# manuelbb-upb/Morbit.jl

Hardware: AMD Instinct MI355X
Metric: RBF build+solve+eval cycles/sec (higher is better)
Workload: dtype f64

## Files before the change

include/mrbf.h:

```cpp
#ifndef MRBF_H
#define MRBF_H

#include <stdint.h>

#ifdef __cplusplus
extern "C" {
#endif

typedef struct mrbf_ctx mrbf_ctx;
typedef struct mrbf_model mrbf_model;

enum {
    MRBF_CUBIC = 0,
    MRBF_INV_MULTIQUADRIC = 1,
    MRBF_MULTIQUADRIC = 2,
    MRBF_THIN_PLATE_SPLINE = 3,
    MRBF_GAUSSIAN = 4
};

enum {
    MRBF_OK = 0,
    MRBF_ENOTPD = 1,
    MRBF_ESINGULAR = 2,
    MRBF_EHIP = 3,
// ... 151 lines not shown
    const double *X;
    double *weights_out;
    double *poly_out;
    double *vals_out;
    double *jac_out;
} mrbf_problem;

typedef struct {
    int32_t status;
    int32_t device;
    mrbf_fit_info fit;
    float ms_eval;
    double checksum_w;
    double checksum_vals;
} mrbf_result;

int32_t mrbf_batch_run(int32_t n_dev, const int32_t *device_ids, int64_t n_problems, const mrbf_problem *problems,
                       mrbf_result *results);

typedef struct {
    int64_t n;
    int32_t d, k, kernel_id, poly_deg;
    double a, b;
    const double *centres, *values;
    double *weights_out, *poly_out;
    mrbf_model *model;
    int32_t status;
    int32_t reserved;
    mrbf_fit_info info;
} mrbf_fit_job;
int32_t mrbf_fit_batch(mrbf_ctx *ctx, int64_t n_starts, mrbf_fit_job *jobs, float *ms_total);

typedef struct {
    const mrbf_model *model;
    int64_t m;
    const double *X;
    double *vals_out;
    double *jac_out;
    int32_t status;
    int32_t reserved;
} mrbf_eval_job;
int32_t mrbf_eval_batch(mrbf_ctx *ctx, int64_t n_jobs, mrbf_eval_job *jobs, float *ms_total);
int32_t mrbf_eval_batch_limited(mrbf_ctx *ctx, int64_t n_jobs, mrbf_eval_job *jobs, float *ms_total, int64_t arena_limit_bytes);

typedef struct {
    const mrbf_model *model;
    int64_t m;
    const double *X;
    const int32_t *rows;
    double *hess_out;
    int32_t n_rows;
    int32_t status;
    int32_t nsplit;
    int32_t reserved;
} mrbf_hess_job;
typedef struct {
    float ms_total;
    int32_t chunks;
    int32_t groups;
    int32_t single_inside;
} mrbf_hess_batch_info;
int32_t mrbf_eval_hessian_batch(mrbf_ctx *ctx, int64_t n_jobs, mrbf_hess_job *jobs, mrbf_hess_batch_info *info);
int32_t mrbf_eval_hessian_batch_limited(mrbf_ctx *ctx, int64_t n_jobs, mrbf_hess_job *jobs, mrbf_hess_batch_info *info,
                                        int64_t arena_limit_bytes);

typedef struct mrbf_db mrbf_db;
int32_t mrbf_db_create(mrbf_ctx *ctx, int32_t d, int32_t k, int64_t capacity_hint, mrbf_db **db);
int32_t mrbf_db_append(mrbf_ctx *ctx, mrbf_db *db, int64_t m, const double *sites, const double *values, int64_t *first_index);
int32_t mrbf_db_set_values(mrbf_ctx *ctx, mrbf_db *db, int64_t m, const int64_t *indices, const double *values);
int32_t mrbf_db_read(mrbf_ctx *ctx, const mrbf_db *db, int64_t first, int64_t m, double *sites_out, double *values_out);
int32_t mrbf_db_dims(const mrbf_db *db, int64_t *n_sites, int32_t *d, int32_t *k);
int32_t mrbf_db_free(mrbf_ctx *ctx, mrbf_db *db);

typedef struct {
    mrbf_db *db;
    const double *lb, *ub, *x0;
    int64_t n_exclude;
    const int64_t *exclude;
    int32_t zero_first_pick;
    int32_t rc;
    int64_t *indices_out;
    double *sites_out, *shifted_out;
    double *first_row;
    int64_t mc;
    int64_t first_pick;
    const double *cand_sites_dev;
    const double *shifted_dev;
} mrbf_db_box_job;
int32_t mrbf_db_box_batch(mrbf_ctx *ctx, int64_t n_starts, int32_t d, int32_t p_is_inf, mrbf_db_box_job *jobs, float *ms_total);

typedef struct {
    mrbf_db *db;
    int64_t n_idx;
    const int64_t *indices;
    double *sites_out, *values_out;
    const double *sites_dev;
    const double *values_dev;
    int32_t rc;
    int32_t reserved;
} mrbf_db_gather_job;
int32_t mrbf_db_gather_batch(mrbf_ctx *ctx, int64_t n_starts, int32_t d, mrbf_db_gather_job *jobs, float *ms_total);

typedef struct {
    mrbf_db *db;
    int64_t m;
    const double *sites;
    const double *values;
    int64_t first_index;
    int32_t rc;
    int32_t reserved;
} mrbf_db_append_job;
int32_t mrbf_db_append_batch(mrbf_ctx *ctx, int64_t n_starts, mrbf_db_append_job *jobs, float *ms_total);
typedef struct {
    mrbf_db *db;
    int64_t m;
    const int64_t *indices;
    const double *values;
    int32_t rc;
    int32_t reserved;
} mrbf_db_set_values_job;
int32_t mrbf_db_set_values_batch(mrbf_ctx *ctx, int64_t n_starts, mrbf_db_set_values_job *jobs, float *ms_total);

enum { MRBF_R3_UPDATE = 0, MRBF_R3_IMPROVE = 1 };
enum { MRBF_R3_DONE = 0, MRBF_R3_REBUILT = 1 };
typedef struct {
    mrbf_db *db;
    const double *x, *lb, *ub;
    double pivot_val;
    const double *dirs;
    int32_t n_dirs, reversed;
    int32_t n_missing, max_new;
    int32_t ensure_fully_linear, force_rebuild, mode;
    int32_t rc;
    double *new_sites_out;
    int64_t first_index;
    int32_t n_new, fully_linear, status, n_dirs_used;
} mrbf_round3_job;
int32_t mrbf_db_round3_batch(mrbf_ctx *ctx, int64_t n_starts, int32_t d, mrbf_round3_job *jobs, float *ms_total);

int32_t mrbf_debug_env(const char *name);
int32_t mrbf_debug_mfma_layout(mrbf_ctx *ctx, double *out16x16_a_times_b, const double *A16x4, const double *B4x16);
int32_t mrbf_debug_potrf(mrbf_ctx *ctx, int64_t n, double *A_colmajor_inout, int32_t impl, int32_t *info, float *ms);
int32_t mrbf_debug_diag(mrbf_ctx *ctx, const double *A128, int32_t reps, float *ms_per_call, double *shader_cycles,
                        double *realtime_us);
int32_t mrbf_debug_mfma_peak(mrbf_ctx *ctx, int32_t blocks_per_cu, int32_t threads, int32_t iters, float *ms, double *tflops);
int32_t mrbf_debug_mfma_asm(mrbf_ctx *ctx, int32_t variant, int32_t blocks_per_cu, int32_t iters, float *ms, double *tflops,
                            double *cycles_per_mfma);
int32_t mrbf_debug_dgemm(mrbf_ctx *ctx, int32_t m, int32_t n, int32_t k, float *ms, double *tflops);
int32_t mrbf_debug_mega_tables(int32_t nt, int32_t mt, int32_t slack, int32_t slack_chain, int32_t first, int32_t win, int32_t srows,
                               int32_t half_cols, int64_t *out6);
int32_t mrbf_debug_mega_tables2(int32_t nt, int32_t mt, int32_t slack, int32_t slack_chain, int32_t first, int32_t win, int32_t srows,
                                int32_t half_cols, const int32_t *opt5, int64_t *out6);
int32_t mrbf_debug_mega_plan(int32_t nt, int32_t mt, int32_t xreal, int64_t *out39);

enum { MRBF_PS_OK = 0, MRBF_PS_CRITICAL = 1, MRBF_PS_FAILURE = 2 };
typedef struct {
    int32_t max_ideal_evals;
    int32_t max_ps_evals;
    int32_t max_polish_evals;
    int32_t reserved;
    uint64_t seed;
    double t0;
    double xtol_rel;
} mrbf_ps_options;
typedef struct {
    int32_t status;
    int32_t generations;
    int32_t evals_ideal, evals_ps, evals_polish;
    float ms_total;
    double tau;
} mrbf_ps_info;
int32_t mrbf_ps_step(mrbf_ctx *ctx, const mrbf_model *model, const double *x_n, const double *lb_eff, const double *ub_eff,
                     const double *fx_n, const double *r_or_null, const mrbf_ps_options *opts, double *x_trial, double *mx_trial,
                     double *r_out, mrbf_ps_info *info);

enum { MRBF_ROLE_NONE = -1, MRBF_ROLE_EQ = -2, MRBF_ROLE_INEQ = -3 };
typedef struct {
    int32_t n_models, n_objectives;
    const mrbf_model *const *models;
    const int32_t *roles;
    int32_t n_lin_eq, n_lin_ineq;
    const double *A_eq, *b_eq, *A_ineq, *b_ineq;
    double eq_tol;
} mrbf_ps_problem;
int32_t mrbf_ps_step_problem(mrbf_ctx *ctx, const mrbf_ps_problem *problem, const double *x_n, const double *lb_eff,
                             const double *ub_eff, const double *fx_n, const double *r_or_null, const mrbf_ps_options *opts,
                             double *x_trial, double *mx_trial, double *r_out, mrbf_ps_info *info);
int32_t mrbf_debug_ps_rank(mrbf_ctx *ctx, int32_t lam, const double *f, const double *phi, uint64_t seed, int32_t gen, int32_t impl,
                           int32_t *order_out, int32_t *gave_up);

enum { MRBF_SD_OK = 0, MRBF_SD_NO_OBJECTIVE = 1, MRBF_SD_INFEASIBLE = 2, MRBF_SD_GAVE_UP = 3 };
int32_t mrbf_sd_direction(mrbf_ctx *ctx, int64_t n_lp, int32_t d, int32_t k, int32_t m_eq, int32_t m_ineq, const double *G,
                          const double *x, const double *lb, const double *ub, const double *A_eq, const double *b_eq,
                          const double *A_ineq, const double *b_ineq, int32_t normalize, double *d_out, double *omega_out,
                          double *dual_out, int32_t *status_out, int32_t *iters_out);
typedef struct {
    int32_t status;
    int32_t iterations;
    int32_t bound_flips;
    float ms_total;
    double omega;
} mrbf_sd_info;
int32_t mrbf_sd_criticality(mrbf_ctx *ctx, const mrbf_ps_problem *problem, const double *x, const double *x_n, const double *lb,
                            const double *ub, int32_t normalize, double *d_out, double *dual_out, mrbf_sd_info *info);

enum { MRBF_NS_OK = 0, MRBF_NS_INFEASIBLE = 1, MRBF_NS_GAVE_UP = 2 };
int32_t mrbf_normal_direction(mrbf_ctx *ctx, int64_t n_lp, int32_t d, int32_t m_eq, int32_t m_ineq, const double *x, const double *lb,
                              const double *ub, const double *A_eq, const double *b_eq, const double *A_ineq, const double *b_ineq,
                              double *n_out, double *alpha_out, double *dual_out, int32_t *status_out, int32_t *iters_out);
typedef struct {
    int32_t status;
    int32_t iterations;
    int32_t bound_flips;
    float ms_total;
    double alpha;
    double delta;
} mrbf_normal_info;
int32_t mrbf_normal_step(mrbf_ctx *ctx, const mrbf_ps_problem *problem, int32_t d, const double *x, const double *lb, const double *ub,
                         double delta, double kappa_delta, double delta_max, int32_t variable_radius, double *n_out, double *dual_out,
                         mrbf_normal_info *info);

typedef struct {
    int32_t strict;
    int32_t max_loops;
    double const_rhs;
    double shrink;
    double min_stepsize;
} mrbf_sd_step_options;
typedef struct {
    int32_t branch;
    int32_t loops;
    float ms_total;
    double sigma;
    double omega;
    double step_norm;
} mrbf_sd_step_info;
int32_t mrbf_sd_step(mrbf_ctx *ctx, const mrbf_ps_problem *problem, const double *x, const double *x_n, double delta, const double *lb,
                     const double *ub, double omega, const double *d, const mrbf_sd_step_options *opts, double *x_plus, double *mx_plus,
                     mrbf_sd_step_info *info);

typedef struct {
    int32_t sd_status;
    int32_t iterations, bound_flips;
    int32_t branch, loops;
    int32_t reserved;
    double omega;
    double omega_step;
    double sigma, step_norm;
} mrbf_sd_batch_record;
int32_t mrbf_sd_iterate_batch(mrbf_ctx *ctx, int64_t n_starts, const mrbf_ps_problem *shape, const mrbf_model *const *models,
                              const double *x, const double *x_n, const double *delta, const double *lb, const double *ub,
                              int32_t normalize, const mrbf_sd_step_options *opts, double *d_out, double *x_plus, double *mx_plus,
                              mrbf_sd_batch_record *records, float *ms_total);

typedef struct {
    int32_t status;
    int32_t iterations, bound_flips;
    int32_t reserved;
    double alpha;
    double delta;
} mrbf_normal_batch_record;
int32_t mrbf_normal_step_batch(mrbf_ctx *ctx, int64_t n_starts, const mrbf_ps_problem *shape, const mrbf_model *const *models, int32_t d,
                               const double *x, const double *lb, const double *ub, const double *delta, double kappa_delta,
                               double delta_max, int32_t variable_radius, double *n_out, double *x_n_out, double *dual_out,
                               mrbf_normal_batch_record *records, float *ms_total);

int32_t mrbf_ps_step_batch(mrbf_ctx *ctx, int64_t n_starts, const mrbf_ps_problem *shape, const mrbf_model *const *models,
                           const double *x_n, const double *lb_eff, const double *ub_eff, const double *fx_n, const double *r_or_null,
                           const mrbf_ps_options *opts, const uint64_t *seeds_or_null, double *x_trial, double *mx_trial, double *r_out,
                           mrbf_ps_info *infos, float *ms_total);

enum { MRBF_DISPATCH_REFERENCE = 0, MRBF_DISPATCH_DEVICE = 1 };
enum { MRBF_FIT_FULL = 0, MRBF_FIT_FROM_ROUND4 = 1 };
enum { MRBF_ENTRY_ROUND4 = 1, MRBF_ENTRY_FIT_FROM_ROUND4 = 2, MRBF_ENTRY_PS_STEP = 3, MRBF_ENTRY_BACKTRACK = 4, MRBF_ENTRY_AFFINE = 5,
       MRBF_ENTRY_SD = 6, MRBF_ENTRY_NORMAL = 7, MRBF_ENTRY_SD_STEP = 8, MRBF_ENTRY_SD_BATCH = 9, MRBF_ENTRY_AFFINE_BATCH = 10,
       MRBF_ENTRY_FIT_BATCH = 11, MRBF_ENTRY_NORMAL_BATCH = 12, MRBF_ENTRY_ROUND4_BATCH = 13, MRBF_ENTRY_PS_BATCH = 14,
       MRBF_ENTRY_DB_BOX = 15, MRBF_ENTRY_DB_GATHER = 16, MRBF_ENTRY_DB_ROUND3 = 17, MRBF_ENTRY_DB_APPEND_BATCH = 18,
       MRBF_ENTRY_DB_SET_VALUES_BATCH = 19, MRBF_ENTRY_EVAL_BATCH = 20, MRBF_ENTRY_HESSIAN_BATCH = 21 };
int32_t mrbf_dispatch_ps(int32_t d, int32_t k, int32_t n_models, int32_t n_nl_constraints, int32_t n_lin_constraints, int32_t n_foreign);
int32_t mrbf_dispatch_ps_batch(int64_t n_starts, int32_t d, int32_t k, int32_t n_models, int32_t n_nl_constraints,
                               int32_t n_lin_constraints, int32_t n_foreign);
int32_t mrbf_dispatch_sd(int32_t d, int32_t k, int32_t n_models, int32_t n_nl_constraints, int32_t n_lin_constraints, int32_t n_foreign);
int32_t mrbf_dispatch_normal(int32_t d, int32_t n_models, int32_t n_nl_constraints, int32_t n_lin_constraints, int32_t n_foreign);
int32_t mrbf_dispatch_sd_step(int32_t d, int32_t k, int32_t n_models, int32_t n_nl_constraints, int32_t n_lin_constraints, int32_t n_foreign,
                              int32_t max_loops);
int32_t mrbf_dispatch_sd_batch(int64_t n_starts, int32_t d, int32_t k, int32_t n_models, int32_t n_nl_constraints,
                               int32_t n_lin_constraints, int32_t n_foreign, int32_t max_loops);
int32_t mrbf_dispatch_normal_batch(int64_t n_starts, int32_t d, int32_t n_models, int32_t n_nl_constraints, int32_t n_lin_constraints,
                                   int32_t n_foreign);
int32_t mrbf_dispatch_backtrack(int32_t n_objective_models, int32_t n_foreign, int32_t outputs_in_order);
int32_t mrbf_dispatch_affine(int64_t n_candidates, int32_t d);
int32_t mrbf_dispatch_affine_batch(int64_t n_starts, int32_t d, int32_t p_is_inf);
int32_t mrbf_dispatch_round4(int64_t n0, int32_t d, int32_t poly_deg, int64_t n_candidates);
int32_t mrbf_dispatch_fit_batch(int64_t n_starts);
int64_t mrbf_dispatch_fit_batch_max_n(int64_t n_starts, int32_t d);
int32_t mrbf_dispatch_fit_batch_lu(int64_t n_lu_starts, int64_t n_max, int32_t d);
int32_t mrbf_dispatch_round4_batch(int64_t n_starts, int32_t d);
int32_t mrbf_dispatch_db_batch(int64_t n_starts, int32_t d);
int32_t mrbf_dispatch_eval_batch(int64_t n_jobs);
int64_t mrbf_dispatch_eval_batch_min_jobs(void);
int32_t mrbf_dispatch_hessian_batch(int64_t n_jobs);
int64_t mrbf_dispatch_hessian_batch_min_jobs(void);
int32_t mrbf_dispatch_fit(int64_t n_training, int64_t state_n0, int32_t state_q, int32_t state_n_accepted, int32_t same_sites);
int32_t mrbf_dispatch_after(int32_t entry, int32_t rc);

int32_t mrbf_stochastic_rank(int32_t lam, const double *f, const double *phi, const double *u, double pf, int32_t *idx_out);
// ... 6 lines not shown
```

morbit.jl_amd/_lib.py:

```python
import ctypes
import os

import numpy as np

_HERE = os.path.dirname(os.path.abspath(__file__))
LIB_PATH = os.environ.get("MRBF_LIB") or os.path.join(_HERE, "libmrbf.so")

c_dp = ctypes.POINTER(ctypes.c_double)
c_fp = ctypes.POINTER(ctypes.c_float)
c_ip = ctypes.POINTER(ctypes.c_int32)
c_vp = ctypes.c_void_p

MRBF_OK, MRBF_ENOTPD, MRBF_ESINGULAR, MRBF_EHIP, MRBF_EBLAS, MRBF_ENOMEM, MRBF_ENODEVICE, MRBF_ENCCL = range(8)
PATH_CHOL, PATH_PROJ_CHOL, PATH_LU, PATH_MINNORM, PATH_ROUND4 = 1, 2, 3, 4, 5
OPT_GRAM_MODE, OPT_RESIDUAL, OPT_FORCE_PATH, OPT_CHOL_IMPL, OPT_EVAL_IMPL, OPT_TIMING, OPT_DIAG_IMPL, OPT_CHOL_WINDOW = 1, 2, 3, 4, 5, 6, 7, 8
OPT_SPIN_MS, OPT_DEBUG_FAULT, OPT_LAST_DEVICE_MS, OPT_SLOW_LAUNCHES = 9, 10, 11, 12
OPT_ARENA_BYTES, OPT_LIVE_HANDLES = 13, 14
OPT_SMALL_FIT_MAX_N = 15
SMALL_FIT_DEFAULT_MAX_N = 512
OPT_SMALL_LU = 16
SMALL_LU_MAX_N, SMALL_LU_MAX_D, SMALL_LU_MAX_K = 512, 128, 16
FB_CHOL_HOST_DRIVEN, FB_BACKSOLVE_BLOCKED, FB_LU = 1, 2, 4


# ... 126 lines not shown

    def asdict(self):
        return {f: getattr(self, f) for f, _ in self._fields_}


class AffineJob(ctypes.Structure):
    _fields_ = [("mc", ctypes.c_int64), ("j0", ctypes.c_int32), ("max_picks", ctypes.c_int32), ("pivot_val", ctypes.c_double),
                ("shifted", ctypes.c_void_p), ("Q0", ctypes.c_void_p), ("picked_out", ctypes.c_void_p), ("Z_out", ctypes.c_void_p),
                ("n_picked", ctypes.c_int32), ("reserved", ctypes.c_int32)]


class Round4Job(ctypes.Structure):
    _fields_ = [("n0", ctypes.c_int64), ("mc", ctypes.c_int64), ("start_sites", ctypes.c_void_p), ("cand_sites", ctypes.c_void_p),
                ("kernel_id", ctypes.c_int32), ("poly_deg", ctypes.c_int32), ("a", ctypes.c_double), ("b", ctypes.c_double),
                ("max_points", ctypes.c_int32), ("theta_pivot_cholesky", ctypes.c_double), ("accepted_out", ctypes.c_void_p),
                ("n_accepted", ctypes.c_int32), ("rc", ctypes.c_int32)]


class FitJob(ctypes.Structure):
    _fields_ = [("n", ctypes.c_int64), ("d", ctypes.c_int32), ("k", ctypes.c_int32), ("kernel_id", ctypes.c_int32),
                ("poly_deg", ctypes.c_int32), ("a", ctypes.c_double), ("b", ctypes.c_double), ("centres", ctypes.c_void_p),
                ("values", ctypes.c_void_p), ("weights_out", ctypes.c_void_p), ("poly_out", ctypes.c_void_p), ("model", ctypes.c_void_p),
                ("status", ctypes.c_int32), ("reserved", ctypes.c_int32), ("info", FitInfo)]


class EvalJob(ctypes.Structure):
    _fields_ = [("model", ctypes.c_void_p), ("m", ctypes.c_int64), ("X", ctypes.c_void_p), ("vals_out", ctypes.c_void_p),
                ("jac_out", ctypes.c_void_p), ("status", ctypes.c_int32), ("reserved", ctypes.c_int32)]


class DbBoxJob(ctypes.Structure):
    _fields_ = [("db", ctypes.c_void_p), ("lb", ctypes.c_void_p), ("ub", ctypes.c_void_p), ("x0", ctypes.c_void_p),
                ("n_exclude", ctypes.c_int64), ("exclude", ctypes.c_void_p), ("zero_first_pick", ctypes.c_int32), ("rc", ctypes.c_int32),
                ("indices_out", ctypes.c_void_p), ("sites_out", ctypes.c_void_p), ("shifted_out", ctypes.c_void_p),
                ("first_row", ctypes.c_void_p), ("mc", ctypes.c_int64), ("first_pick", ctypes.c_int64),
                ("cand_sites_dev", ctypes.c_void_p), ("shifted_dev", ctypes.c_void_p)]


class DbGatherJob(ctypes.Structure):
    _fields_ = [("db", ctypes.c_void_p), ("n_idx", ctypes.c_int64), ("indices", ctypes.c_void_p), ("sites_out", ctypes.c_void_p),
                ("values_out", ctypes.c_void_p), ("sites_dev", ctypes.c_void_p), ("values_dev", ctypes.c_void_p),
                ("rc", ctypes.c_int32), ("reserved", ctypes.c_int32)]


class DbAppendJob(ctypes.Structure):
    _fields_ = [("db", ctypes.c_void_p), ("m", ctypes.c_int64), ("sites", ctypes.c_void_p), ("values", ctypes.c_void_p),
                ("first_index", ctypes.c_int64), ("rc", ctypes.c_int32), ("reserved", ctypes.c_int32)]


class DbSetValuesJob(ctypes.Structure):
    _fields_ = [("db", ctypes.c_void_p), ("m", ctypes.c_int64), ("indices", ctypes.c_void_p), ("values", ctypes.c_void_p),
                ("rc", ctypes.c_int32), ("reserved", ctypes.c_int32)]


class Round3Job(ctypes.Structure):
    _fields_ = [("db", ctypes.c_void_p), ("x", ctypes.c_void_p), ("lb", ctypes.c_void_p), ("ub", ctypes.c_void_p),
                ("pivot_val", ctypes.c_double), ("dirs", ctypes.c_void_p), ("n_dirs", ctypes.c_int32), ("reversed", ctypes.c_int32),
                ("n_missing", ctypes.c_int32), ("max_new", ctypes.c_int32), ("ensure_fully_linear", ctypes.c_int32),
                ("force_rebuild", ctypes.c_int32), ("mode", ctypes.c_int32), ("rc", ctypes.c_int32), ("new_sites_out", ctypes.c_void_p),
                ("first_index", ctypes.c_int64), ("n_new", ctypes.c_int32), ("fully_linear", ctypes.c_int32), ("status", ctypes.c_int32),
                ("n_dirs_used", ctypes.c_int32)]


class Problem(ctypes.Structure):
    _fields_ = [("n", ctypes.c_int64), ("m", ctypes.c_int64), ("d", ctypes.c_int32), ("k", ctypes.c_int32),
                ("kernel_id", ctypes.c_int32), ("poly_deg", ctypes.c_int32), ("a", ctypes.c_double), ("b", ctypes.c_double),
                ("centres", c_dp), ("values", c_dp), ("X", c_dp), ("weights_out", c_dp), ("poly_out", c_dp),
                ("vals_out", c_dp), ("jac_out", c_dp)]


class Result(ctypes.Structure):
    _fields_ = [("status", ctypes.c_int32), ("device", ctypes.c_int32), ("fit", FitInfo), ("ms_eval", ctypes.c_float),
                ("checksum_w", ctypes.c_double), ("checksum_vals", ctypes.c_double)]


SIGNATURES = {
    "mrbf_init": (ctypes.c_int32, [ctypes.c_int32, ctypes.POINTER(c_vp)]),
    "mrbf_shutdown": (ctypes.c_int32, [c_vp]),
    "mrbf_last_error": (ctypes.c_char_p, [c_vp]),
    "mrbf_version": (ctypes.c_char_p, []),
    "mrbf_set_option": (ctypes.c_int32, [c_vp, ctypes.c_int32, ctypes.c_double]),
    "mrbf_get_option": (ctypes.c_int32, [c_vp, ctypes.c_int32, c_dp]),
    "mrbf_set_stream": (ctypes.c_int32, [c_vp, c_vp]),
    "mrbf_sync": (ctypes.c_int32, [c_vp]),
    "mrbf_gram": (ctypes.c_int32, [c_vp, ctypes.c_int64, ctypes.c_int32, c_vp, ctypes.c_int32, ctypes.c_double,
                                   ctypes.c_double, ctypes.c_int32, c_vp, c_vp, c_fp]),
    "mrbf_cross_gram": (ctypes.c_int32, [c_vp, ctypes.c_int64, ctypes.c_int64, ctypes.c_int32, c_vp, c_vp, ctypes.c_int32, ctypes.c_double,
                                         ctypes.c_double, c_vp]),
    "mrbf_fit": (ctypes.c_int32, [c_vp, ctypes.c_int64, ctypes.c_int32, ctypes.c_int32, c_vp, c_vp, ctypes.c_int32,
                                  ctypes.c_double, ctypes.c_double, ctypes.c_int32, ctypes.POINTER(c_vp), c_vp, c_vp,
                                  ctypes.POINTER(FitInfo)]),
    "mrbf_model_from_coeffs": (ctypes.c_int32, [c_vp, ctypes.c_int64, ctypes.c_int32, ctypes.c_int32, c_vp, c_vp, c_vp,
                                                ctypes.c_int32, ctypes.c_double, ctypes.c_double, ctypes.c_int32,
                                                ctypes.POINTER(c_vp)]),
    "mrbf_eval": (ctypes.c_int32, [c_vp, c_vp, ctypes.c_int64, c_vp, c_vp, c_vp, ctypes.POINTER(EvalInfo)]),
    "mrbf_eval_hessian": (ctypes.c_int32, [c_vp, c_vp, ctypes.c_int64, c_vp, ctypes.c_int32, c_vp, c_vp, ctypes.POINTER(HessInfo)]),
    "mrbf_eval_hessian_limited": (ctypes.c_int32, [c_vp, c_vp, ctypes.c_int64, c_vp, ctypes.c_int32, c_vp, c_vp, ctypes.POINTER(HessInfo),
                                                   ctypes.c_int64]),
    "mrbf_backtrack": (ctypes.c_int32, [c_vp, c_vp, c_vp, c_vp, ctypes.c_double, ctypes.c_double, ctypes.c_int32,
                                        ctypes.c_double, ctypes.c_double, ctypes.c_double, ctypes.c_int32, c_vp, c_vp,
                                        c_vp, c_ip]),
    "mrbf_affine_scores": (ctypes.c_int32, [c_vp, ctypes.c_int64, ctypes.c_int32, ctypes.c_int32, c_vp, c_vp, ctypes.c_int32, c_vp,
                                            ctypes.POINTER(ctypes.c_int64), c_dp]),
    "mrbf_affine_select": (ctypes.c_int32, [c_vp, ctypes.c_int64, ctypes.c_int32, c_vp, ctypes.c_int32, c_vp, ctypes.c_int32, ctypes.c_double,
                                            ctypes.c_int32, ctypes.POINTER(ctypes.c_int64), c_ip, c_vp]),
    "mrbf_affine_select_batch": (ctypes.c_int32, [c_vp, ctypes.c_int64, ctypes.c_int32, ctypes.c_int32, ctypes.POINTER(AffineJob), c_fp]),
    "mrbf_round4": (ctypes.c_int32, [c_vp, ctypes.c_int64, ctypes.c_int32, c_vp, ctypes.c_int64, c_vp, ctypes.c_int32, ctypes.c_double,
                                     ctypes.c_double, ctypes.c_int32, ctypes.c_int32, ctypes.c_double, c_vp, c_ip, ctypes.POINTER(c_vp)]),
    "mrbf_fit_from_round4": (ctypes.c_int32, [c_vp, c_vp, ctypes.c_int32, c_vp, ctypes.POINTER(c_vp), c_vp, c_vp, ctypes.POINTER(FitInfo)]),
    "mrbf_round4_sites": (ctypes.c_int32, [c_vp, ctypes.POINTER(ctypes.c_int64), ctypes.POINTER(ctypes.c_int64), c_ip]),
    "mrbf_free_round4": (ctypes.c_int32, [c_vp, c_vp]),
    "mrbf_round4_batch": (ctypes.c_int32, [c_vp, ctypes.c_int64, ctypes.c_int32, ctypes.POINTER(Round4Job), c_fp]),
    "mrbf_dispatch_round4_batch": (ctypes.c_int32, [ctypes.c_int64, ctypes.c_int32]),
    "mrbf_model_dims": (ctypes.c_int32, [c_vp, ctypes.POINTER(ctypes.c_int64), c_ip, c_ip, c_ip]),
    "mrbf_free_model": (ctypes.c_int32, [c_vp, c_vp]),
    "mrbf_batch_run": (ctypes.c_int32, [ctypes.c_int32, c_ip, ctypes.c_int64, ctypes.POINTER(Problem),
                                        ctypes.POINTER(Result)]),
    "mrbf_fit_batch": (ctypes.c_int32, [c_vp, ctypes.c_int64, ctypes.POINTER(FitJob), c_fp]),
    "mrbf_dispatch_fit_batch": (ctypes.c_int32, [ctypes.c_int64]),
    "mrbf_dispatch_fit_batch_max_n": (ctypes.c_int64, [ctypes.c_int64, ctypes.c_int32]),
    "mrbf_dispatch_fit_batch_lu": (ctypes.c_int32, [ctypes.c_int64, ctypes.c_int64, ctypes.c_int32]),
    "mrbf_eval_batch": (ctypes.c_int32, [c_vp, ctypes.c_int64, ctypes.POINTER(EvalJob), c_fp]),
    "mrbf_eval_batch_limited": (ctypes.c_int32, [c_vp, ctypes.c_int64, ctypes.POINTER(EvalJob), c_fp, ctypes.c_int64]),
    "mrbf_dispatch_eval_batch": (ctypes.c_int32, [ctypes.c_int64]),
    "mrbf_dispatch_eval_batch_min_jobs": (ctypes.c_int64, []),
    "mrbf_eval_hessian_batch": (ctypes.c_int32, [c_vp, ctypes.c_int64, ctypes.POINTER(HessJob), ctypes.POINTER(HessBatchInfo)]),
    "mrbf_eval_hessian_batch_limited": (ctypes.c_int32, [c_vp, ctypes.c_int64, ctypes.POINTER(HessJob), ctypes.POINTER(HessBatchInfo),
                                                         ctypes.c_int64]),
    "mrbf_dispatch_hessian_batch": (ctypes.c_int32, [ctypes.c_int64]),
    "mrbf_dispatch_hessian_batch_min_jobs": (ctypes.c_int64, []),
    "mrbf_db_create": (ctypes.c_int32, [c_vp, ctypes.c_int32, ctypes.c_int32, ctypes.c_int64, ctypes.POINTER(c_vp)]),
    "mrbf_db_append": (ctypes.c_int32, [c_vp, c_vp, ctypes.c_int64, c_vp, c_vp, ctypes.POINTER(ctypes.c_int64)]),
    "mrbf_db_set_values": (ctypes.c_int32, [c_vp, c_vp, ctypes.c_int64, c_vp, c_vp]),
    "mrbf_db_read": (ctypes.c_int32, [c_vp, c_vp, ctypes.c_int64, ctypes.c_int64, c_vp, c_vp]),
    "mrbf_db_dims": (ctypes.c_int32, [c_vp, ctypes.POINTER(ctypes.c_int64), c_ip, c_ip]),
    "mrbf_db_free": (ctypes.c_int32, [c_vp, c_vp]),
    "mrbf_db_box_batch": (ctypes.c_int32, [c_vp, ctypes.c_int64, ctypes.c_int32, ctypes.c_int32, ctypes.POINTER(DbBoxJob), c_fp]),
    "mrbf_db_gather_batch": (ctypes.c_int32, [c_vp, ctypes.c_int64, ctypes.c_int32, ctypes.POINTER(DbGatherJob), c_fp]),
    "mrbf_db_append_batch": (ctypes.c_int32, [c_vp, ctypes.c_int64, ctypes.POINTER(DbAppendJob), c_fp]),
    "mrbf_db_set_values_batch": (ctypes.c_int32, [c_vp, ctypes.c_int64, ctypes.POINTER(DbSetValuesJob), c_fp]),
    "mrbf_db_round3_batch": (ctypes.c_int32, [c_vp, ctypes.c_int64, ctypes.c_int32, ctypes.POINTER(Round3Job), c_fp]),
    "mrbf_dispatch_db_batch": (ctypes.c_int32, [ctypes.c_int64, ctypes.c_int32]),
    "mrbf_debug_mfma_layout": (ctypes.c_int32, [c_vp, c_vp, c_vp, c_vp]),
    "mrbf_debug_potrf": (ctypes.c_int32, [c_vp, ctypes.c_int64, c_vp, ctypes.c_int32, c_ip, c_fp]),
    "mrbf_debug_env": (ctypes.c_int32, [ctypes.c_char_p]),
    "mrbf_debug_diag": (ctypes.c_int32, [c_vp, c_vp, ctypes.c_int32, c_fp, c_dp, c_dp]),
    "mrbf_debug_ps_rank": (ctypes.c_int32, [c_vp, ctypes.c_int32, c_vp, c_vp, ctypes.c_uint64, ctypes.c_int32, ctypes.c_int32, c_ip, c_ip]),
    "mrbf_debug_mfma_peak": (ctypes.c_int32, [c_vp, ctypes.c_int32, ctypes.c_int32, ctypes.c_int32, c_fp, c_dp]),
    "mrbf_debug_mfma_asm": (ctypes.c_int32, [c_vp, ctypes.c_int32, ctypes.c_int32, ctypes.c_int32, c_fp, c_dp, c_dp]),
    "mrbf_debug_dgemm": (ctypes.c_int32, [c_vp, ctypes.c_int32, ctypes.c_int32, ctypes.c_int32, c_fp, c_dp]),
    "mrbf_debug_mega_tables": (ctypes.c_int32, [ctypes.c_int32] * 8 + [c_vp]),
    "mrbf_debug_mega_tables2": (ctypes.c_int32, [ctypes.c_int32] * 8 + [c_vp, c_vp]),
    "mrbf_debug_mega_plan": (ctypes.c_int32, [ctypes.c_int32] * 3 + [c_vp]),
    "mrbf_stochastic_rank": (ctypes.c_int32, [ctypes.c_int32, c_vp, c_vp, c_vp, ctypes.c_double, c_vp]),
    "mrbf_ps_step": (ctypes.c_int32, [c_vp, c_vp, c_vp, c_vp, c_vp, c_vp, c_vp, ctypes.POINTER(PsOptions), c_vp, c_vp, c_vp,
                                      ctypes.POINTER(PsInfo)]),
    "mrbf_ps_step_problem": (ctypes.c_int32, [c_vp, ctypes.POINTER(PsProblem), c_vp, c_vp, c_vp, c_vp, c_vp, ctypes.POINTER(PsOptions),
                                              c_vp, c_vp, c_vp, ctypes.POINTER(PsInfo)]),
    "mrbf_ps_step_batch": (ctypes.c_int32, [c_vp, ctypes.c_int64, ctypes.POINTER(PsProblem), ctypes.POINTER(ctypes.c_void_p), c_vp, c_vp, c_vp,
                                            c_vp, c_vp, ctypes.POINTER(PsOptions), ctypes.POINTER(ctypes.c_uint64), c_vp, c_vp, c_vp,
                                            ctypes.POINTER(PsInfo), c_fp]),
    "mrbf_dispatch_ps_batch": (ctypes.c_int32, [ctypes.c_int64] + [ctypes.c_int32] * 6),
    "mrbf_sd_direction": (ctypes.c_int32, [c_vp, ctypes.c_int64, ctypes.c_int32, ctypes.c_int32, ctypes.c_int32, ctypes.c_int32] + [c_vp] * 8
                          + [ctypes.c_int32, c_vp, c_vp, c_vp, c_vp, c_vp]),
    "mrbf_sd_criticality": (ctypes.c_int32, [c_vp, ctypes.POINTER(PsProblem), c_vp, c_vp, c_vp, c_vp, ctypes.c_int32, c_vp, c_vp,
                                             ctypes.POINTER(SdInfo)]),
    "mrbf_normal_direction": (ctypes.c_int32, [c_vp, ctypes.c_int64, ctypes.c_int32, ctypes.c_int32, ctypes.c_int32] + [c_vp] * 12),
    "mrbf_normal_step": (ctypes.c_int32, [c_vp, ctypes.POINTER(PsProblem), ctypes.c_int32, c_vp, c_vp, c_vp, ctypes.c_double, ctypes.c_double,
                                          ctypes.c_double, ctypes.c_int32, c_vp, c_vp, ctypes.POINTER(NormalInfo)]),
    "mrbf_sd_step": (ctypes.c_int32, [c_vp, ctypes.POINTER(PsProblem), c_vp, c_vp, ctypes.c_double, c_vp, c_vp, ctypes.c_double, c_vp,
                                      ctypes.POINTER(SdStepOptions), c_vp, c_vp, ctypes.POINTER(SdStepInfo)]),
    "mrbf_sd_iterate_batch": (ctypes.c_int32, [c_vp, ctypes.c_int64, ctypes.POINTER(PsProblem), ctypes.POINTER(ctypes.c_void_p), c_vp, c_vp, c_vp,
                                               c_vp, c_vp, ctypes.c_int32, ctypes.POINTER(SdStepOptions), c_vp, c_vp, c_vp,
                                               ctypes.POINTER(SdBatchRecord), c_fp]),
    "mrbf_dispatch_sd_batch": (ctypes.c_int32, [ctypes.c_int64] + [ctypes.c_int32] * 7),
    "mrbf_normal_step_batch": (ctypes.c_int32, [c_vp, ctypes.c_int64, ctypes.POINTER(PsProblem), ctypes.POINTER(ctypes.c_void_p), ctypes.c_int32,
                                                c_vp, c_vp, c_vp, c_vp, ctypes.c_double, ctypes.c_double, ctypes.c_int32, c_vp, c_vp, c_vp,
                                                ctypes.POINTER(NormalBatchRecord), c_fp]),
    "mrbf_dispatch_normal_batch": (ctypes.c_int32, [ctypes.c_int64] + [ctypes.c_int32] * 5),
    "mrbf_dispatch_ps": (ctypes.c_int32, [ctypes.c_int32] * 6),
    "mrbf_dispatch_sd_step": (ctypes.c_int32, [ctypes.c_int32] * 7),
    "mrbf_dispatch_sd": (ctypes.c_int32, [ctypes.c_int32] * 6),
    "mrbf_dispatch_normal": (ctypes.c_int32, [ctypes.c_int32] * 5),
    "mrbf_dispatch_backtrack": (ctypes.c_int32, [ctypes.c_int32] * 3),
    "mrbf_dispatch_affine": (ctypes.c_int32, [ctypes.c_int64, ctypes.c_int32]),
    "mrbf_dispatch_affine_batch": (ctypes.c_int32, [ctypes.c_int64, ctypes.c_int32, ctypes.c_int32]),
    "mrbf_dispatch_round4": (ctypes.c_int32, [ctypes.c_int64, ctypes.c_int32, ctypes.c_int32, ctypes.c_int64]),
    "mrbf_dispatch_fit": (ctypes.c_int32, [ctypes.c_int64, ctypes.c_int64, ctypes.c_int32, ctypes.c_int32, ctypes.c_int32]),
    "mrbf_dispatch_after": (ctypes.c_int32, [ctypes.c_int32, ctypes.c_int32]),
}

_LIB = None


class MrbfError(RuntimeError):
    def __init__(self, code, msg):
        super().__init__("libmrbf error %d: %s" % (code, msg))
        self.code = code


def load():
    global _LIB
    if _LIB is None:
        if not os.path.exists(LIB_PATH):
            raise ImportError("libmrbf.so is not built (%s); run `python -c 'import __graft_entry__ as g; g.build()'` "
                              "or `make -C morbit.jl_amd/csrc`. There is no CPU fallback." % LIB_PATH)
        lib = ctypes.CDLL(LIB_PATH)
        for name, (res, args) in SIGNATURES.items():
            fn = getattr(lib, name)
            fn.restype = res
            fn.argtypes = args
        _LIB = lib
    return _LIB


def as_ptr(a):
    if a is None:
        return None
    if isinstance(a, np.ndarray):
        return ctypes.c_void_p(a.ctypes.data)
    if hasattr(a, "data_ptr"):
        return ctypes.c_void_p(a.data_ptr())
    raise TypeError("expected numpy array or tensor, got %r" % type(a))


def host_f64(a, shape=None):
    a = np.ascontiguousarray(a, dtype=np.float64)
    if shape is not None:
        a = a.reshape(shape)
    return a


class Context:

    def __init__(self, device_id=-1):
        self.lib = load()
        h = c_vp()
        rc = self.lib.mrbf_init(device_id, ctypes.byref(h))
        if rc != 0:
            raise MrbfError(rc, (self.lib.mrbf_last_error(None) or b"").decode())
        self.h = h

    def check(self, rc):
        if rc != 0:
            raise MrbfError(rc, (self.lib.mrbf_last_error(self.h) or b"").decode())

    def set_option(self, key, value):
        self.check(self.lib.mrbf_set_option(self.h, key, float(value)))

    def get_option(self, key):
        v = ctypes.c_double()
        self.check(self.lib.mrbf_get_option(self.h, key, ctypes.byref(v)))
        return v.value

    def sync(self):
        self.check(self.lib.mrbf_sync(self.h))

    def close(self):
        if getattr(self, "h", None):
            self.lib.mrbf_shutdown(self.h)
            self.h = None

    def __del__(self):
        try:
            self.close()
        except Exception:
            pass


_DEFAULT_CTX = {}


def default_context(device_id=-1):
    import threading

    key = (threading.get_ident(), device_id)
    if key not in _DEFAULT_CTX:
        _DEFAULT_CTX[key] = Context(device_id)
    return _DEFAULT_CTX[key]
```

morbit.jl_amd/csrc/chol.hip:

```cpp
#include <chrono>

#include "common.hpp"

namespace mrbf {

int debug_diag(mrbf_ctx *ctx, const double *A128_dev, int reps, float *ms_per_call, unsigned long long *stamps_host);
int launch_pad_identity(mrbf_ctx *ctx, double *A, int64_t n, int64_t npad, int64_t ld);

int potrf_lower(mrbf_ctx *ctx, int impl, int64_t n, double *A, int64_t lda, int *info_host) {
    int *dinfo;
    MRBF_TRY(get_buf(ctx, S_INFO, (size_t)4, &dinfo));
    const int64_t npad = round_up(n, 128);
    if (impl == 0) impl = (lda >= npad) ? ((npad >= ctx->mega.min && npad <= ctx->mega.max) ? 3 : 2) : 1;
    if (impl == 2 || impl == 3) {
        if (lda < npad) return fail(ctx, MRBF_EHIP, "built-in Cholesky needs lda >= round_up(n,128)");
        MRBF_TRY(launch_pad_identity(ctx, A, n, npad, lda));
        PotrfOpts opt;
        opt.impl = impl;
        opt.any_size = true;
        MRBF_TRY(potrf_blocked_tall(ctx, npad, npad, A, lda, dinfo, nullptr, opt));
    } else {
        MRBF_BLAS(ctx, rocsolver_dpotrf(ctx->blas, rocblas_fill_lower, (int)n, A, (int)lda, dinfo));
    }
    MRBF_HIP(ctx, hipMemcpyAsync(info_host, dinfo, sizeof(int), hipMemcpyDeviceToHost, ctx->stream));
    MRBF_HIP(ctx, hipStreamSynchronize(ctx->stream));
    MRBF_TRY(mega_collect_stat(ctx));
    return 0;
}

}

using namespace mrbf;

extern "C" int32_t mrbf_debug_potrf(mrbf_ctx *ctx, int64_t n, double *A, int32_t impl, int32_t *info, float *ms) {
    if (!ctx) return -1;
    if (n <= 0) return -2;
    if (!A) return -3;
    (void)hipSetDevice(ctx->device);
    const int64_t npad = round_up(n, 128);
    double *dA;
    MRBF_TRY(get_buf(ctx, S_PHI, (size_t)npad * npad, &dA));
    const hipMemcpyKind in = is_device_ptr(A) ? hipMemcpyDeviceToDevice : hipMemcpyHostToDevice;
    const hipMemcpyKind out = is_device_ptr(A) ? hipMemcpyDeviceToDevice : hipMemcpyDeviceToHost;
    MRBF_HIP(ctx, hipMemcpy2DAsync(dA, (size_t)npad * sizeof(double), A, (size_t)n * sizeof(double), (size_t)n * sizeof(double),
                                   (size_t)n, in, ctx->stream));
    int hinfo = 0;
    static const double host_trace_ms = mrbf_env("MRBF_MEGA_HOSTTRACE") ? atof(mrbf_env("MRBF_MEGA_HOSTTRACE")) : 0.0;
    auto now_ms = []() { return std::chrono::duration<double, std::milli>(std::chrono::steady_clock::now().time_since_epoch()).count(); };
    const double h0 = now_ms();
    MRBF_HIP(ctx, hipEventRecord(ctx->ev[0], ctx->stream));
    const double h1 = now_ms();
    MRBF_TRY(potrf_lower(ctx, impl, n, dA, npad, &hinfo));
    const double h2 = now_ms();
    MRBF_HIP(ctx, hipEventRecord(ctx->ev[1], ctx->stream));
    MRBF_HIP(ctx, hipEventSynchronize(ctx->ev[1]));
    const double h3 = now_ms();
    if (host_trace_ms > 0.0 && h3 - h0 > host_trace_ms)
        fprintf(stderr, "mrbf_debug_potrf host trace (n %lld): record ev0 %.3f ms | potrf_lower incl. sync %.3f | record ev1 + sync %.3f\n", (long long)n,
                h1 - h0, h2 - h1, h3 - h2);
    if (ms) MRBF_HIP(ctx, hipEventElapsedTime(ms, ctx->ev[0], ctx->ev[1]));
    if (info) *info = hinfo;
    MRBF_HIP(ctx, hipMemcpy2DAsync(A, (size_t)n * sizeof(double), dA, (size_t)npad * sizeof(double), (size_t)n * sizeof(double),
                                   (size_t)n, out, ctx->stream));
    MRBF_HIP(ctx, hipStreamSynchronize(ctx->stream));
    return MRBF_OK;
}

extern "C" int32_t mrbf_debug_diag(mrbf_ctx *ctx, const double *A128, int32_t reps, float *ms_per_call, double *shader_cycles,
                                   double *realtime_us) {
    if (!ctx) return -1;
    if (!A128) return -2;
    (void)hipSetDevice(ctx->device);
    const double *dA;
    MRBF_TRY(stage_in(ctx, S_STAGE_A, A128, 128 * 128, &dA));
    unsigned long long st[6] = {0, 0, 0, 0, 0, 0};
    float ms = 0;
    MRBF_TRY(debug_diag(ctx, dA, reps, &ms, st));
    if (ms_per_call) *ms_per_call = ms;
    if (shader_cycles) *shader_cycles = (double)st[0];
    if (realtime_us) *realtime_us = (double)st[1] / 100.0;
    if (mrbf_env("MRBF_DIAG_VERBOSE"))
        fprintf(stderr, "diag segments (cycles over 128 columns, wave 0): barrier %llu read %llu critical %llu rest %llu\n", st[2], st[3],
                st[4], st[5]);
    return MRBF_OK;
}
```

morbit.jl_amd/csrc/chol_blocked.hip:

```cpp
#include "common.hpp"
#include "mega_gemm.hpp"

namespace mrbf {

typedef double v4d __attribute__((ext_vector_type(4)));
typedef double v2d __attribute__((ext_vector_type(2)));

constexpr int CNB = 128;

enum { UPD_LOWER_SUB = 0, UPD_OVERWRITE = 1, UPD_FULL_SUB = 2, UPD_COLUMN_SUB = 3 };
int launch_diag(mrbf_ctx *ctx, hipStream_t st, double *Ajj, int64_t lda, double *Linv, int *dinfo, int col0);

template <int TM, int MODE>
__global__ __launch_bounds__(256, 2) void chol_update_kernel(const double *__restrict__ A, int64_t lda,
                                                             const double *__restrict__ B, int64_t ldb,
                                                             double *__restrict__ C, int64_t ldc, int K,
                                                             const int *__restrict__ info, int mt_sq = 0, int ntiles_total = 0,
                                                             const double *__restrict__ cvec = nullptr, double cs = 0.0, int64_t cn = 0) {
    constexpr int NJ = (TM == 128) ? 4 : 2;
    __shared__ __attribute__((aligned(16))) double smem[mega::NSTG * mega::STG];
    if (info && *info != 0) return;
    if (MODE == UPD_OVERWRITE || MODE == UPD_COLUMN_SUB) __builtin_amdgcn_s_setprio(2);
    const int tid = threadIdx.x, lane = tid & 63, wave = tid >> 6;
    const int l15 = lane & 15, l4 = lane >> 4;
    const int tile_end = (MODE == UPD_LOWER_SUB && ntiles_total > 0) ? ntiles_total : (int)blockIdx.x + 1;
    for (int bid = blockIdx.x; bid < tile_end; bid += gridDim.x) {
    int ti, tj;
    if (MODE == UPD_LOWER_SUB) {
        const int ntri = mt_sq * (mt_sq + 1) / 2;
        if (bid < ntri || mt_sq == 0) {
            int t = (int)((sqrt(8.0 * (double)bid + 1.0) - 1.0) * 0.5);
            while ((t + 1) * (t + 2) / 2 <= bid) ++t;
            while (t * (t + 1) / 2 > bid) --t;
            ti = t;
            tj = bid - t * (t + 1) / 2;
        } else {
            ti = mt_sq + (bid - ntri) / mt_sq;
            tj = (bid - ntri) % mt_sq;
        }
    } else {
        ti = blockIdx.x;
        tj = blockIdx.y;
    }
    const int64_t I0 = (int64_t)ti * TM, J0 = (int64_t)tj * 128;
    const int ioff = (TM == 128) ? (wave >> 1) * 64 : 0;
    const int joff = (TM == 128) ? (wave & 1) * 64 : wave * 32;

    v4d acc[NJ][4];
#pragma unroll
    for (int j = 0; j < NJ; ++j)
#pragma unroll
        for (int i = 0; i < 4; ++i) acc[j][i] = (v4d){0.0, 0.0, 0.0, 0.0};

    asm volatile("s_waitcnt vmcnt(0)" ::: "memory");
    constexpr bool NEG_START = (MODE == UPD_LOWER_SUB);
    if (NEG_START) {
#pragma unroll
        for (int j = 0; j < NJ; ++j)
#pragma unroll
            for (int r = 0; r < 4; ++r) {
                const int64_t gj = J0 + joff + j * 16 + l4 + 4 * r;
#pragma unroll
                for (int i = 0; i < 4; ++i) acc[j][i][r] = -C[(I0 + ioff + i * 16 + l15) + gj * ldc];
            }
    }
    mega::gemm_acc<TM>(A + I0, lda, B + J0, ldb, K, acc, smem);
    double cvi[4] = {0.0, 0.0, 0.0, 0.0}, cei[4] = {0.0, 0.0, 0.0, 0.0};
    if (MODE == UPD_LOWER_SUB && cvec) {
#pragma unroll
        for (int i = 0; i < 4; ++i) {
            const int64_t gi = I0 + ioff + i * 16 + l15;
            cvi[i] = cs * cvec[gi];
            cei[i] = gi < cn ? cs : 0.0;
        }
    }
#pragma unroll
    for (int j = 0; j < NJ; ++j) {
        double cv[4][4];
        double cvj[4] = {0.0, 0.0, 0.0, 0.0}, cej[4] = {0.0, 0.0, 0.0, 0.0};
        if (MODE == UPD_LOWER_SUB && cvec) {
#pragma unroll
            for (int r = 0; r < 4; ++r) {
                const int64_t gj = J0 + joff + j * 16 + l4 + 4 * r;
                cvj[r] = cvec[gj];
                cej[r] = gj < cn ? 1.0 : 0.0;
            }
        }
        if (MODE != UPD_OVERWRITE && !NEG_START) {
#pragma unroll
            for (int r = 0; r < 4; ++r) {
                const int64_t gj = J0 + joff + j * 16 + l4 + 4 * r;
#pragma unroll
                for (int i = 0; i < 4; ++i) cv[r][i] = C[(I0 + ioff + i * 16 + l15) + gj * ldc];
            }
        }
#pragma unroll
        for (int r = 0; r < 4; ++r) {
            const int64_t gj = J0 + joff + j * 16 + l4 + 4 * r;
#pragma unroll
            for (int i = 0; i < 4; ++i) {
                const int64_t gi = I0 + ioff + i * 16 + l15;
                double *dst = C + gi + gj * ldc;
                if (MODE == UPD_OVERWRITE) {
                    *dst = acc[j][i][r];
                } else if (MODE == UPD_FULL_SUB) {
                    *dst = cv[r][i] - acc[j][i][r];
                } else if (MODE == UPD_COLUMN_SUB) {
                    if (gi >= gj) *dst = cv[r][i] - acc[j][i][r];
                } else {
                    double x = -acc[j][i][r];
                    if (cvec) x -= fma(cei[i], cvj[r], cvi[i] * cej[r]);
                    if (ti != tj || gi >= gj) *dst = x;
                }
            }
        }
    }
    if (bid + (int)gridDim.x < tile_end) __syncthreads();
    }
}

struct __attribute__((aligned(16))) DiagShared {
    double col[2][2 * CNB];
    double rinv[2];
    int sbad;
    unsigned long long seg[4];
    int stamp;
};

__device__ __forceinline__ double fast_rsqrt(double x) {
    double y = __builtin_amdgcn_rsq(x);
    const double h = 0.5 * x;
#pragma unroll
    for (int it = 0; it < 3; ++it) y = y * fma(-h, y * y, 1.5);
    return y;
}

template <int KV, bool STAMP>
__device__ __forceinline__ void diag_phase(double (&a)[8][8], DiagShared &sh, int ti, int tj, int half, int &buf, int &bad) {
    constexpr int KN = (KV < 7) ? KV + 1 : 7;
    double piv = 0.0;
    if (half == 0) piv = __shfl(a[KV][KV], tj, 16);
#pragma unroll 1
    for (int kk = 0; kk < 16; ++kk) {
        const int k = KV * 16 + kk;
        const bool st = STAMP && threadIdx.x < 64;
        unsigned long long s0 = 0, s1 = 0, s2 = 0, s3 = 0;
        if (st) s0 = __builtin_amdgcn_s_memtime();
        __syncthreads();
        if (st) s1 = __builtin_amdgcn_s_memtime();
        double lj[8];
#pragma unroll
        for (int v = KV; v < 8; ++v) lj[v] = sh.col[buf][tj + 16 * v];
        if (half == 0) {
            double li[8];
#pragma unroll
            for (int u = KV; u < 8; ++u) li[u] = sh.col[buf][ti + 16 * u];
            if (st) {
                asm volatile("s_waitcnt lgkmcnt(0)" ::: "memory");
                s2 = __builtin_amdgcn_s_memtime();
            }
            if (kk < 15) {
                if (tj > kk) piv = fma(-lj[KV], lj[KV], piv);
                if (tj == kk + 1) {
                    const int kn = k + 1;
                    double rinv = 0.0;
                    if (piv > 0.0) {
                        rinv = fast_rsqrt(piv);
                    } else if (bad == 0) {
                        bad = kn + 1;
                    }
                    if (ti == 0) sh.rinv[buf ^ 1] = rinv;
                    double w[8];
#pragma unroll
                    for (int u = 0; u < 8; ++u) {
                        const int i = ti + 16 * u;
                        double val = 0.0;
                        if (u >= KV && i >= kn) {
                            val = fma(-li[u], lj[KV], a[u][KV]) * rinv;
                            a[u][KV] = val;
                        }
                        w[u] = val;
                    }
#pragma unroll
                    for (int u = 0; u < 8; ++u) sh.col[buf ^ 1][ti + 16 * u] = w[u];
                }
            } else if (KV < 7) {
                if (tj == 0) {
                    const int kn = k + 1;
// ... 48 lines not shown
#pragma unroll
            for (int u = 0; u <= KV; ++u) {
                const double erk = sh.col[buf][CNB + ti + 16 * u] * rinv;
                if (tj == kk) a[u][KV] = erk;
                a[u][KV] = fma(-erk, ljk, a[u][KV]);
#pragma unroll
                for (int v = KV + 1; v < 8; ++v) a[u][v] = fma(-erk, lj[v], a[u][v]);
            }
            if (kk < 15) {
                if (tj == kk + 1) {
#pragma unroll
                    for (int u = 0; u < 8; ++u) sh.col[buf ^ 1][CNB + ti + 16 * u] = (u <= KV) ? a[u][KV] : 0.0;
                }
            } else if (KV < 7) {
                if (tj == 0) {
#pragma unroll
                    for (int u = 0; u < 8; ++u) sh.col[buf ^ 1][CNB + ti + 16 * u] = (u <= KN) ? a[u][KN] : 0.0;
                }
            }
        }
        buf ^= 1;
    }
}

template <bool STAMP>
__global__ __launch_bounds__(512) void chol_diag_kernel(double *__restrict__ A, int64_t lda, double *__restrict__ Linv,
                                                        int *__restrict__ info, int col0,
                                                        unsigned long long *__restrict__ stamps) {
    __shared__ DiagShared sh;
    if (*info != 0) return;
    unsigned long long t0 = 0, r0 = 0;
    if (STAMP) {
        if (threadIdx.x == 0) sh.seg[0] = sh.seg[1] = sh.seg[2] = sh.seg[3] = 0;
        __syncthreads();
        t0 = __builtin_amdgcn_s_memtime();
        r0 = __builtin_amdgcn_s_memrealtime();
    }
    const int tid = threadIdx.x, ti = tid & 15, tj = (tid >> 4) & 15, half = tid >> 8;
    double a[8][8];
#pragma unroll
    for (int v = 0; v < 8; ++v)
#pragma unroll
        for (int u = 0; u < 8; ++u) {
            const int i = ti + 16 * u, j = tj + 16 * v;
            if (half == 0)
                a[u][v] = (i >= j) ? A[i + (int64_t)j * lda] : 0.0;
            else
                a[u][v] = (i == j) ? 1.0 : 0.0;
        }
    int buf = 0, bad = 0;
    if (tj == 0) {
        if (half == 0) {
            const double pv = __shfl(a[0][0], 0, 16);
            double rinv = 0.0;
            if (pv > 0.0) {
                rinv = fast_rsqrt(pv);
            } else {
                bad = 1;
            }
            if (ti == 0) sh.rinv[0] = rinv;
#pragma unroll
            for (int u = 0; u < 8; ++u) {
                a[u][0] *= rinv;
                sh.col[0][ti + 16 * u] = a[u][0];
            }
        } else {
#pragma unroll
            for (int u = 0; u < 8; ++u) sh.col[0][CNB + ti + 16 * u] = (u == 0) ? a[0][0] : 0.0;
        }
    }
    diag_phase<0, STAMP>(a, sh, ti, tj, half, buf, bad);
    diag_phase<1, STAMP>(a, sh, ti, tj, half, buf, bad);
    diag_phase<2, STAMP>(a, sh, ti, tj, half, buf, bad);
    diag_phase<3, STAMP>(a, sh, ti, tj, half, buf, bad);
    diag_phase<4, STAMP>(a, sh, ti, tj, half, buf, bad);
    diag_phase<5, STAMP>(a, sh, ti, tj, half, buf, bad);
    diag_phase<6, STAMP>(a, sh, ti, tj, half, buf, bad);
    diag_phase<7, STAMP>(a, sh, ti, tj, half, buf, bad);
    if (tid == 0) sh.sbad = 0x7fffffff;
    __syncthreads();
    if (bad) atomicMin(&sh.sbad, bad);
    __syncthreads();
    if (sh.sbad != 0x7fffffff) {
        if (tid == 0) *info = col0 + sh.sbad;
        return;
    }
#pragma unroll
    for (int v = 0; v < 8; ++v)
#pragma unroll
        for (int u = 0; u < 8; ++u) {
            const int i = ti + 16 * u, j = tj + 16 * v;
            if (half == 0) {
                if (i >= j) A[i + (int64_t)j * lda] = a[u][v];
            } else {
                Linv[j + i * CNB] = (j >= i) ? a[u][v] : 0.0;
            }
        }
    if (STAMP && threadIdx.x == 0) {
        stamps[0] = __builtin_amdgcn_s_memtime() - t0;
        stamps[1] = __builtin_amdgcn_s_memrealtime() - r0;
        for (int q = 0; q < 4; ++q) stamps[2 + q] = sh.seg[q];
    }
}

__global__ void pad_identity_kernel(double *__restrict__ A, int64_t n, int64_t npad, int64_t ld) {
    const int64_t idx = (int64_t)blockIdx.x * blockDim.x + threadIdx.x;
    const int64_t pw = npad - n;
    if (idx >= npad * pw) return;
    const int64_t j = n + idx / npad, i = idx % npad;
    A[i + j * ld] = (i == j) ? 1.0 : 0.0;
    if (i < n) A[j + i * ld] = 0.0;
}

int launch_pad_identity(mrbf_ctx *ctx, double *A, int64_t n, int64_t npad, int64_t ld) {
    if (npad == n) return 0;
    const int64_t cnt = npad * (npad - n);
    hipLaunchKernelGGL(pad_identity_kernel, dim3((unsigned)((cnt + 255) / 256)), dim3(256), 0, ctx->stream, A, n, npad, ld);
    MRBF_HIP(ctx, hipGetLastError());
    return 0;
}

int debug_diag(mrbf_ctx *ctx, const double *A128_dev, int reps, float *ms_per_call, unsigned long long *stamps_host) {
    const bool with_stamps = reps > 0;
    if (reps < 0) reps = -reps;
    double *W, *Linv;
    int *dinfo;
    unsigned long long *st;
    MRBF_TRY(get_buf(ctx, S_PHI, (size_t)CNB * CNB * reps, &W));
    MRBF_TRY(get_buf(ctx, S_CHOL_WS, (size_t)CNB * CNB, &Linv));
    MRBF_TRY(get_buf(ctx, S_INFO, (size_t)4, &dinfo));
    MRBF_TRY(get_buf(ctx, S_MISC, (size_t)8, (double **)&st));
    for (int r = 0; r < reps; ++r)
        MRBF_HIP(ctx, hipMemcpyAsync(W + (size_t)r * CNB * CNB, A128_dev, sizeof(double) * CNB * CNB, hipMemcpyDeviceToDevice, ctx->stream));
    MRBF_HIP(ctx, hipMemsetAsync(dinfo, 0, sizeof(int), ctx->stream));
    MRBF_HIP(ctx, hipEventRecord(ctx->ev[0], ctx->stream));
    for (int r = 0; r < reps; ++r)
        if (ctx->diag_impl != 1)
            launch_diag(ctx, ctx->stream, W + (size_t)r * CNB * CNB, (int64_t)CNB, Linv, dinfo, 0);
        else if (with_stamps)
            hipLaunchKernelGGL(chol_diag_kernel<true>, dim3(1), dim3(512), 0, ctx->stream, W + (size_t)r * CNB * CNB, (int64_t)CNB, Linv,
                               dinfo, 0, st);
        else
            hipLaunchKernelGGL(chol_diag_kernel<false>, dim3(1), dim3(512), 0, ctx->stream, W + (size_t)r * CNB * CNB, (int64_t)CNB, Linv,
                               dinfo, 0, (unsigned long long *)nullptr);
    MRBF_HIP(ctx, hipEventRecord(ctx->ev[1], ctx->stream));
    MRBF_HIP(ctx, hipEventSynchronize(ctx->ev[1]));
    float t;
    MRBF_HIP(ctx, hipEventElapsedTime(&t, ctx->ev[0], ctx->ev[1]));
    *ms_per_call = t / reps;
    MRBF_HIP(ctx, hipMemcpy(stamps_host, st, 6 * sizeof(unsigned long long), hipMemcpyDeviceToHost));
    return 0;
}

int launch_update_lower(mrbf_ctx *ctx, const double *A, int64_t lda, const double *B, int64_t ldb, double *C, int64_t ldc, int64_t nt,
                        int K, const double *cvec, double cs, int64_t cn) {
    if (nt <= 0 || K <= 0) return 0;
    hipLaunchKernelGGL((chol_update_kernel<128, UPD_LOWER_SUB>), dim3((unsigned)(nt * (nt + 1) / 2)), dim3(256), 0, ctx->stream, A,
                       lda, B, ldb, C, ldc, K, (const int *)nullptr, (int)nt, 0, cvec, cs, cn);
    MRBF_HIP(ctx, hipGetLastError());
    return 0;
}

int potrf_blocked_tall(mrbf_ctx *ctx, int64_t ncols, int64_t mrows, double *A, int64_t lda, int *dinfo, double *linv_all, PotrfOpts opt) {
    if (ncols % CNB != 0 || mrows % CNB != 0 || mrows < ncols || (lda & 1) || (reinterpret_cast<uintptr_t>(A) & 15))
        return fail(ctx, MRBF_EHIP, "potrf_blocked needs 128-padded, 16-byte aligned storage (ncols=%lld mrows=%lld lda=%lld)",
                    (long long)ncols, (long long)mrows, (long long)lda);
    const int impl = opt.impl != 0 ? opt.impl : ctx->chol_impl;
    if ((impl == 3 || (impl == 0 && ncols <= ctx->mega.max)) && (opt.any_size || ncols >= ctx->mega.min))
        return potrf_mega_tall(ctx, ncols, mrows, A, lda, dinfo, linv_all, opt);
    double *Lone = nullptr;
    if (!linv_all) MRBF_TRY(get_buf(ctx, S_CHOL_WS, (size_t)CNB * CNB, &Lone));
    hipStream_t S = ctx->stream, M = ctx->bulk_stream, P = ctx->panel_stream;
    hipEvent_t evStart = ctx->evx[0], evT = ctx->evx[1], evU2 = ctx->evx[2], evEnd = ctx->evx[3];
    const bool single = ncols <= 4 * CNB;
    if (single) M = P = S;
    MRBF_HIP(ctx, hipMemsetAsync(dinfo, 0, sizeof(int), S));
    if (!single) {
        MRBF_HIP(ctx, hipEventRecord(evStart, S));
        MRBF_HIP(ctx, hipStreamWaitEvent(P, evStart, 0));
        MRBF_HIP(ctx, hipStreamWaitEvent(M, evStart, 0));
    }
    const int nb = (int)(ncols / CNB);
    bool have_u2 = false;
    int w0 = 0, W = 1;
    for (int j = 0; j < nb; ++j) {
        const int64_t c = (int64_t)j * CNB;
        if (j == w0) {
            const int64_t rem = ncols - c;
            W = (rem > 4800) ? 4 : (rem > 2400 ? 2 : 1);
            if (ctx->chol_window > 0) W = ctx->chol_window;
        }
        const bool last_in_window = (j == w0 + W - 1) || (j == nb - 1);
        const int kpan = (int)((j - w0 + 1) * CNB);
        const int64_t cw = (int64_t)w0 * CNB;
        double *Ajj = A + c + c * lda;
        double *Linv = linv_all ? linv_all + (size_t)j * CNB * CNB : Lone;
        if (ctx->diag_impl == 1)
            hipLaunchKernelGGL(chol_diag_kernel<false>, dim3(1), dim3(512), 0, P, Ajj, lda, Linv, dinfo, (int)c,
                               (unsigned long long *)nullptr);
        else
            launch_diag(ctx, P, Ajj, lda, Linv, dinfo, (int)c);
        const int64_t m = mrows - c - CNB;
        if (m <= 0) break;
        double *A21 = A + (c + CNB) + c * lda;
        hipLaunchKernelGGL((chol_update_kernel<64, UPD_OVERWRITE>), dim3((unsigned)(m / 64), 1), dim3(256), 0, P, A21, lda, Linv,
                           (int64_t)CNB, A21, lda, CNB, dinfo);
        if (c + CNB >= ncols) break;
        if (!single) MRBF_HIP(ctx, hipEventRecord(evT, P));
        if (have_u2 && !single) {
            MRBF_HIP(ctx, hipStreamWaitEvent(P, evU2, 0));
            have_u2 = false;
        }
        const double *Pw = A + (c + CNB) + cw * lda;
        double *A22 = A + (c + CNB) + (c + CNB) * lda;
        hipLaunchKernelGGL((chol_update_kernel<64, UPD_COLUMN_SUB>), dim3((unsigned)(m / 64), 1), dim3(256), 0, P, Pw, lda, Pw, lda,
                           A22, lda, kpan, dinfo);
        if (last_in_window) {
            const int64_t mt2 = (ncols - c - 2 * CNB) / CNB;
            if (mt2 > 0) {
                if (!single) MRBF_HIP(ctx, hipStreamWaitEvent(M, evT, 0));
                const int64_t mx = (mrows - ncols) / CNB;
                const int64_t rem_next = ncols - c - CNB;
                int Wn = (rem_next > 4800) ? 4 : (rem_next > 2400 ? 2 : 1);
                if (ctx->chol_window > 0) Wn = ctx->chol_window;
                const int64_t na = std::min<int64_t>(Wn, mt2);
                const double *P2 = A + (c + 2 * CNB) + cw * lda;
                double *C2 = A + (c + 2 * CNB) + (c + 2 * CNB) * lda;
                hipLaunchKernelGGL((chol_update_kernel<128, UPD_LOWER_SUB>),
                                   dim3((unsigned)(na * (na + 1) / 2 + (mt2 - na + mx) * na)), dim3(256), 0, M, P2, lda, P2, lda, C2, lda,
                                   kpan, dinfo, (int)na);
                if (!single) MRBF_HIP(ctx, hipEventRecord(evU2, M));
                have_u2 = true;
                const int64_t mb2 = mt2 - na;
                if (mb2 > 0) {
                    const double *P3 = P2 + na * CNB;
                    double *C3 = C2 + na * CNB + na * CNB * lda;
                    const int64_t nt3 = mb2 * (mb2 + 1) / 2 + mx * mb2;
                    const int64_t g3 = (ctx->bulk_grid > 0 && nt3 > ctx->bulk_grid) ? ctx->bulk_grid : nt3;
                    hipLaunchKernelGGL((chol_update_kernel<128, UPD_LOWER_SUB>), dim3((unsigned)g3), dim3(256), 0, M, P3, lda, P3, lda,
                                       C3, lda, kpan, dinfo, (int)mb2, (int)nt3);
                }
            }
            w0 = j + 1;
        }
    }
    MRBF_HIP(ctx, hipGetLastError());
    if (!single) {
        MRBF_HIP(ctx, hipEventRecord(evEnd, P));
        MRBF_HIP(ctx, hipStreamWaitEvent(S, evEnd, 0));
        MRBF_HIP(ctx, hipEventRecord(evStart, M));
        MRBF_HIP(ctx, hipStreamWaitEvent(S, evStart, 0));
    }
    return 0;
}

constexpr int BS_LD = 65;
template <int KB>
__device__ __forceinline__ void tile_tdot(const double *__restrict__ Tl, int64_t ldt, const double *xs ,
                                          double *res , double *stage ,
                                          double *part ) {
    const int tid = threadIdx.x, c = tid & 127, g = tid >> 7;
    double acc[KB];
#pragma unroll
    for (int l = 0; l < KB; ++l) acc[l] = 0.0;
    for (int h = 0; h < 2; ++h) {
        double v[32];
#pragma unroll
        for (int p = 0; p < 32; ++p) v[p] = Tl[(int64_t)(p * 4 + (tid >> 6)) * ldt + 64 * h + (tid & 63)];
        __syncthreads();
#pragma unroll
        for (int p = 0; p < 32; ++p) stage[(p * 4 + (tid >> 6)) * BS_LD + (tid & 63)] = v[p];
        __syncthreads();
#pragma unroll 8
        for (int r = 0; r < 32; ++r) {
            const double t = stage[c * BS_LD + 32 * g + r];
#pragma unroll
            for (int l = 0; l < KB; ++l) acc[l] = fma(t, xs[l * CNB + 64 * h + 32 * g + r], acc[l]);
        }
    }
#pragma unroll
    for (int l = 0; l < KB; ++l) part[l * 256 + tid] = acc[l];
    __syncthreads();
    if (g == 0) {
#pragma unroll
        for (int l = 0; l < KB; ++l) res[l * CNB + c] = part[l * 256 + c] + part[l * 256 + 128 + c];
    }
}

template <int KB>
__global__ __launch_bounds__(256) void chol_backsolve_kernel(const double *__restrict__ L, int64_t lda, const double *__restrict__ linv_all,
                                                             double *__restrict__ Y, int64_t ldy, int k0, int i ,
                                                             int prologue) {
    __shared__ double xs[KB * CNB];
    __shared__ double res[KB * CNB];
    __shared__ double part[KB * 256];
    __shared__ double stage[CNB * BS_LD];
    const int tid = threadIdx.x;
    const int j = blockIdx.x;
    if (!prologue) {
        for (int t = tid; t < KB * CNB; t += 256) xs[t] = Y[(int64_t)(k0 + t / CNB) * ldy + (int64_t)i * CNB + (t % CNB)];
        __syncthreads();
        tile_tdot<KB>(L + (int64_t)i * CNB + (int64_t)j * CNB * lda, lda, xs, res, stage, part);
        __syncthreads();
        for (int t = tid; t < KB * CNB; t += 256) {
            double *yp = Y + (int64_t)(k0 + t / CNB) * ldy + (int64_t)j * CNB + (t % CNB);
            const double v = *yp - res[t];
            *yp = v;
            xs[t] = v;
        }
        if (j != i - 1) return;
        __syncthreads();
    } else {
        for (int t = tid; t < KB * CNB; t += 256) xs[t] = Y[(int64_t)(k0 + t / CNB) * ldy + (int64_t)i * CNB + (t % CNB)];
// ... 32 lines not shown
```

morbit.jl_amd/csrc/common.hpp:

```cpp
#pragma once
#include <hip/hip_runtime.h>
#include <rocblas/rocblas.h>
#include <rocsolver/rocsolver.h>

#include <cmath>
#include <cstdlib>
#include <cstdint>
#include <cstdio>
#include <cstring>
#include <map>
#include <string>
#include <vector>

#include "../../include/mrbf.h"
#include "descent_problem.hpp"
#include "model_pool.hpp"

namespace mrbf {

struct KP {
    int kid;
    double a, b;
    double a2;
    double sgn;
    int fast;
    int ik;
    double phi0;
};
KP make_kp(int kid, double a, double b);
inline bool kp_nonsmooth(const KP &p) { return (p.kid == MRBF_CUBIC && p.a == 1.0) || (p.kid == MRBF_THIN_PLATE_SPLINE && p.ik == 1); }
int cpd_order(int kid, double a, double b);
inline int poly_dim(int d, int deg) { return deg < 0 ? 0 : (deg == 0 ? 1 : d + 1); }

enum Slot {
    S_XC = 0, S_SQ, S_MEAN, S_PHI, S_PI, S_Q1, S_W1, S_G, S_R, S_TAU, S_RHS, S_T1, S_T2, S_IPIV, S_INFO,
    S_STAGE_A, S_STAGE_B, S_STAGE_C, S_STAGE_D, S_EVAL_E, S_EVAL_A, S_EVAL_J, S_EVAL_SA, S_EVAL_XC, S_EVAL_XSQ,
    S_OUT_A, S_OUT_B, S_CHOL_WS, S_MISC, S_MEGA_JOBS, S_MEGA_FLAGS, S_MEGA_WQ, S_MEGA_IT, S_BSOLVE_FLAGS, S_MEGA_TRACE, S_MEGA_JLOG,
    S_T1W, S_PS_STATE, S_PS_STAT, S_PS_POLISH, S_BSOLVE_X, S_V0, S_QR_INV, S_DIAG_SCR, S_SMALL_WS, S_SMALL_DESC, S_SMALL_FLAGS, S_MEGA_STAT, S_BSOLVE_M, S_SMALL_CL, S_GW_PART, S_GW_RS, S_GW_GP, S_GW_M, S_CHECK_SCAL, S_TAIL_PART, S_PS_RANK, S_SD_IN, S_SD_OUT, S_SD_WS, S_NS_IN, S_NS_OUT, S_NS_WS, S_SD_STEP, S_SD_BATCH, S_AFF_BATCH, S_NS_BATCH, S_R4_BATCH, S_DB_BOX, S_DB_GATHER, S_DB_WS, S_SMALL_LU, S_EVAL_BATCH, S_HESS_WS, S_HESS_OUT, S_HESS_BATCH, S_NSLOTS
};
}

namespace mrbf {
namespace mega {
struct Edge {
    int head, tail_c0, srows_edge, pstream_edge;
    int shalf, sh_head, sh_tail_c0;
    int tfull1;
    int xhalf;
};
struct TableParams {
    int slack, slack_chain, first, win, srows, half_cols, tail_half, tail_half_w, chainq;
    Edge edge;
};
constexpr bool operator==(const TableParams &a, const TableParams &b) {
    return a.slack == b.slack && a.slack_chain == b.slack_chain && a.first == b.first && a.win == b.win && a.srows == b.srows &&
           a.half_cols == b.half_cols && a.tail_half == b.tail_half && a.tail_half_w == b.tail_half_w && a.chainq == b.chainq &&
           a.edge.head == b.edge.head && a.edge.tail_c0 == b.edge.tail_c0 && a.edge.srows_edge == b.edge.srows_edge &&
           a.edge.pstream_edge == b.edge.pstream_edge && a.edge.shalf == b.edge.shalf && a.edge.sh_head == b.edge.sh_head &&
           a.edge.sh_tail_c0 == b.edge.sh_tail_c0 && a.edge.tfull1 == b.edge.tfull1 && a.edge.xhalf == b.edge.xhalf;
}
struct Knobs {
    int grid = 512, dedicated = 64, look = 2, quiet = 1, slack = 3, half_cols = 0, first_window = 1, wbias = 4, xhalf = 1, chainq = 0, cboost = 12, panel_dma = 1;
    int min = 256, max = 32768;
    int chain = 0, slack_chain = 0, win = 0, pstream = 0, srows = 0;
    int shalf = -1, shalf_head = -1, head = -1, tail = -1, reserve = -1, tail_half = -1, tail_half_w = -1, xchain = -1, quiet_tail = -1;
    int tfull = -1;
};
}
struct MegaTables {
    int nt, mt;
    mega::TableParams params;
    void *block, *jobs, *wq;
    int npanel, nbulk, nchainjobs, nwin;
    unsigned long long stamp;
};
struct PotrfOpts {
    int impl = 0;
    bool any_size = false;
    int xreal = 0;
    bool info_clean = false;
};
struct EvalHints {
    bool population = false;
    bool check_call = false;
    const double *pre_xq = nullptr;
};
}

struct mrbf_ctx {
    int device = 0;
    int ncu = 256;
    hipStream_t own_stream = nullptr;
    hipStream_t stream = nullptr;
    rocblas_handle blas = nullptr;
    mrbf::Buf slots[mrbf::S_NSLOTS];
    hipEvent_t ev[8] = {};
    hipStream_t panel_stream = nullptr;
    hipEvent_t evx[4] = {};
    hipStream_t bulk_stream = nullptr;
    int bulk_masked = 0;
    int bulk_grid = 384;
    mrbf::mega::Knobs mega;
    std::string err;
    std::vector<mrbf::Buf> model_pool;
    int gram_mode = 0, residual = 1, force_path = 0, chol_impl = 0, eval_impl = 0, timing = 1, diag_impl = 0, chol_window = 0;
    int spin_ms = 1000, debug_fault = 0;
    unsigned long long *mega_stat_dev = nullptr;
    long mega_stat_shape = 0;
    int mega_stat_pending = 0;
    char *pin_base = nullptr;
    size_t pin_off = 0;
    bool pin_armed = false;
    struct PinOut {
        void *user;
        const void *pin;
        size_t bytes;
    };
    std::vector<PinOut> pin_out;
    unsigned long long *hpin = nullptr;
    float last_device_ms = 0.f;
    int slow_launches = 0;
    int small_nc = 4;
    int small_cluster_ok = 0;
    int small_timeouts = 0;
    int small_fit_max_n = 512;
    int small_lu = 0;
    int live_models = 0, live_round4 = 0;
    int live_dbs = 0;
    unsigned ps_rank_epoch = 0;
    int ps_multi_off = 0;
    std::map<long, float> mega_best_ms;
    std::vector<mrbf::MegaTables> mega_tables;
    unsigned long long mega_table_clock = 0;
};

struct mrbf_model {
    int64_t n = 0, npad = 0;
    int d = 0, dpad = 0, k = 0, q = 0, deg = -1;
    mrbf::KP kp{};
    double *C = nullptr;
    double *Xc = nullptr;
    double *sq = nullptr;
    double *mean = nullptr;
    double *W = nullptr;
    double *Wc = nullptr;
    double *lam = nullptr;
    void *block = nullptr;
    size_t block_bytes = 0;
    mrbf_ctx *owner = nullptr;
    mrbf::ModelSlab *slab = nullptr;
};

struct mrbf_db {
    mrbf_ctx *ctx = nullptr;
    int d = 0, k = 0;
    int64_t n = 0, cap = 0;
    double *sites = nullptr, *values = nullptr;
};

namespace mrbf {

int fail(mrbf_ctx *ctx, int code, const char *fmt, ...);
#define MRBF_HIP(ctx, call)                                                                                  \
    do {                                                                                                      \
        hipError_t e__ = (call);                                                                              \
        if (e__ != hipSuccess)                                                                                \
            return mrbf::fail(ctx, e__ == hipErrorOutOfMemory ? MRBF_ENOMEM : MRBF_EHIP, "%s: %s (%s:%d)", #call, \
                              hipGetErrorString(e__), __FILE__, __LINE__);                                    \
    } while (0)
#define MRBF_BLAS(ctx, call)                                                                                 \
    do {                                                                                                      \
        rocblas_status s__ = (call);                                                                          \
        if (s__ != rocblas_status_success)                                                                    \
            return mrbf::fail(ctx, MRBF_EBLAS, "%s: rocblas status %d (%s:%d)", #call, (int)s__, __FILE__, __LINE__); \
    } while (0)
#define MRBF_TRY(call)             \
    do {                           \
        int rc__ = (call);         \
        if (rc__ != 0) return rc__; \
    } while (0)

int get_buf(mrbf_ctx *ctx, Slot s, size_t bytes, void **out);
template <class T>
inline int get_buf(mrbf_ctx *ctx, Slot s, size_t count, T **out) {
    return get_buf(ctx, s, count * sizeof(T), (void **)out);
}
bool is_device_ptr(const void *p);
int db_reserve(mrbf_ctx *ctx, mrbf_db *db, int64_t needed);
int stage_in(mrbf_ctx *ctx, Slot s, const double *user, size_t count, const double **dev);
int stage_out(mrbf_ctx *ctx, Slot s, double *user, size_t count, double **dev);
int finish_out(mrbf_ctx *ctx, double *user, const double *dev, size_t count);
int input_fetch(mrbf_ctx *ctx, const double *src, size_t count, double *dst);
int input_view(mrbf_ctx *ctx, const double *user, size_t count, double *&arena, const double **dev);
int output_put(mrbf_ctx *ctx, double *dst, const double *src, size_t count);
int fetch_linear_rows(mrbf_ctx *ctx, const mrbf_ps_problem *prob, int d, double *A, double *b);
descent::Shape descent_shape(const mrbf_ps_problem *prob, const mrbf_model *const *models, int64_t n_starts,
                             std::vector<descent::SlotShape> &slots);
void pin_reset(mrbf_ctx *ctx);
void pin_flush(mrbf_ctx *ctx);
void pin_discard(mrbf_ctx *ctx);
char *pin_take(mrbf_ctx *ctx, size_t bytes);
struct PinGuard {
    mrbf_ctx *ctx;
    bool flushed = false;
    explicit PinGuard(mrbf_ctx *c) : ctx(c) { pin_reset(c); }
    void flush() {
        pin_flush(ctx);
        flushed = true;
    }
    ~PinGuard() {
        if (!flushed) pin_discard(ctx);
    }
    PinGuard(const PinGuard &) = delete;
    PinGuard &operator=(const PinGuard &) = delete;
};
enum HpinSlot : int {
    HPIN_FIT_FLAGS = 0,
    HPIN_FIT_SCAL = 4,
    HPIN_SMALL_FLAGS = 8,
    HPIN_SMALL_SCAL = 12,
    HPIN_SMALL_CHK = 16,
    HPIN_RESIDUAL = 20,
    HPIN_R4_COUNT = 24,
    HPIN_MEGA_STAT = 63,
};

inline int64_t round_up(int64_t x, int64_t m) { return (x + m - 1) / m * m; }

inline const char *mrbf_env(const char *name) {
    const char *gate = std::getenv("MRBF_EXPERIMENTS");
    if (!gate || std::atoi(gate) == 0) return nullptr;
    return std::getenv(name);
}

int launch_center_pad(mrbf_ctx *ctx, const double *X, int64_t n, int d, const double *mean_or_null, double *mean_out,
                      double *Xc, int64_t npad, int dpad, double *sq);
int launch_poly_matrix(mrbf_ctx *ctx, const double *C, int64_t n, int d, int q, double *Pi, int64_t ldpi);
int launch_transpose(mrbf_ctx *ctx, const double *in, int64_t rows, int64_t cols, double *out);
int launch_gram(mrbf_ctx *ctx, int mode, const double *C, const double *Xc, const double *sq, int64_t n, int64_t npad,
                int d, int dpad, const KP &kp, double *Phi, int64_t ld);
int launch_cross_gram(mrbf_ctx *ctx, const double *X, int64_t m, const double *C, int64_t n, int d, const KP &kp, double *K);
bool gram_w_applies(const mrbf_ctx *ctx, const mrbf_model *M);
int launch_gram_w(mrbf_ctx *ctx, const mrbf_model *M, double *Phi, int64_t ld, double **Wpart_out, double **rspart_out, int *nseg_out);
int launch_projection_small(mrbf_ctx *ctx, const mrbf_model *M, const double *Wpart, const double *rspart, int nseg, const double *linv,
                            const double *Q1, double *W1, double *G, double *scal, int *flags, int K2, int skip, double *PA, double *PB,
                            double *v0);
int eval_model(mrbf_ctx *ctx, const mrbf_model *M, int64_t m, const double *Xdev, double *vals_dev, double *jac_dev,
               mrbf_eval_info *info, EvalHints hints = {});
int hess_call(mrbf_ctx *ctx, const mrbf_model *M, int64_t m, const double *X, const std::vector<int32_t> &rows, double *hess_out,
              mrbf_hess_info *info, int64_t stage_bytes);
int hess_batch_call(mrbf_ctx *ctx, int64_t n_jobs, mrbf_hess_job *jobs, mrbf_hess_batch_info *info, int64_t limit_bytes);
int potrf_blocked_tall(mrbf_ctx *ctx, int64_t ncols, int64_t mrows, double *A, int64_t lda, int *dinfo, double *linv_all, PotrfOpts opt = {});
int potrf_mega_tall(mrbf_ctx *ctx, int64_t ncols, int64_t mrows, double *A, int64_t lda, int *dinfo, double *linv_all, PotrfOpts opt = {});
mega::Knobs mega_knobs_from_env();
int potrf_lower(mrbf_ctx *ctx, int impl, int64_t n, double *A, int64_t lda, int *info_host);
int fit_model(mrbf_ctx *ctx, mrbf_model *M, const double *Ydev, mrbf_fit_info *info);
int build_model_shell(mrbf_ctx *ctx, int64_t n, int d, int k, const double *Cdev, int kid, double a, double b, int deg,
                      mrbf_model **out);
void destroy_model(mrbf_ctx *ctx, mrbf_model *M);
void model_set_dims(mrbf_model *M, int64_t n, int d, int k, int kid, double a, double b, int deg);
size_t model_block_layout(const mrbf_model *M, size_t off[7]);
void model_carve(mrbf_model *M, char *base, const size_t off[7]);
int model_block_acquire(mrbf_ctx *ctx, size_t total, void **p, size_t *bytes);
void model_block_release(mrbf_ctx *ctx, void *p, size_t bytes, bool slab = false);
int fit_check(mrbf_ctx *ctx, mrbf_model *M, const double *Y, mrbf_fit_info *info);
int mega_collect_stat(mrbf_ctx *ctx);
int mega_stat_enqueue(mrbf_ctx *ctx);
int mega_stat_finish(mrbf_ctx *ctx);

}
```

morbit.jl_amd/csrc/context.hip:

```cpp
#include <cstdarg>

#include "common.hpp"

#include <cstring>

namespace mrbf {

static thread_local std::string g_init_err;

int fail(mrbf_ctx *ctx, int code, const char *fmt, ...) {
    char buf[512];
    va_list ap;
    va_start(ap, fmt);
    vsnprintf(buf, sizeof(buf), fmt, ap);
    va_end(ap);
    if (ctx) {
        ctx->err = buf;
    } else {
        g_init_err = buf;
    }
    return code;
}

int cpd_order(int kid, double a, double b) {
// ... 173 lines not shown
    ctx->pin_off = 0;
    ctx->pin_out.clear();
    ctx->pin_armed = true;
}
void pin_flush(mrbf_ctx *ctx) {
    for (const auto &o : ctx->pin_out) std::memcpy(o.user, o.pin, o.bytes);
    ctx->pin_out.clear();
    ctx->pin_armed = false;
}
void pin_discard(mrbf_ctx *ctx) {
    ctx->pin_out.clear();
    ctx->pin_armed = false;
}
char *pin_take(mrbf_ctx *ctx, size_t bytes) {
    if (!ctx->pin_base || !ctx->pin_armed || ctx->pin_off + bytes > PIN_BYTES) return nullptr;
    char *p = ctx->pin_base + ctx->pin_off;
    ctx->pin_off += (bytes + 63) & ~(size_t)63;
    return p;
}

static void mega_stat_account(mrbf_ctx *ctx, unsigned long long ticks);
int mega_stat_enqueue(mrbf_ctx *ctx) {
    if (!ctx->mega_stat_pending || !ctx->mega_stat_dev || !ctx->hpin) return 0;
    ctx->hpin[HPIN_MEGA_STAT] = ~0ull;
    MRBF_HIP(ctx, hipMemcpyAsync(&ctx->hpin[HPIN_MEGA_STAT], ctx->mega_stat_dev, sizeof(unsigned long long), hipMemcpyDeviceToHost, ctx->stream));
    ctx->mega_stat_pending = 2;
    return 0;
}
int mega_stat_finish(mrbf_ctx *ctx) {
    if (ctx->mega_stat_pending != 2) return mega_collect_stat(ctx);
    ctx->mega_stat_pending = 0;
    mega_stat_account(ctx, ctx->hpin[HPIN_MEGA_STAT]);
    return 0;
}
int mega_collect_stat(mrbf_ctx *ctx) {
    if (!ctx->mega_stat_pending || !ctx->mega_stat_dev) return 0;
    ctx->mega_stat_pending = 0;
    unsigned long long ticks = 0;
    MRBF_HIP(ctx, hipMemcpy(&ticks, ctx->mega_stat_dev, sizeof(ticks), hipMemcpyDeviceToHost));
    mega_stat_account(ctx, ticks);
    return 0;
}
static void mega_stat_account(mrbf_ctx *ctx, unsigned long long ticks) {
    const float ms = (float)((double)ticks * 1e-5);
    ctx->last_device_ms = ms;
    if (ms > 0.f) {
        auto it = ctx->mega_best_ms.find(ctx->mega_stat_shape);
        if (it == ctx->mega_best_ms.end()) {
            if (ctx->mega_best_ms.size() > 256) ctx->mega_best_ms.clear();
            ctx->mega_best_ms[ctx->mega_stat_shape] = ms;
        } else {
            if (ms > 2.f * it->second) ++ctx->slow_launches;
            if (ms < it->second) it->second = ms;
        }
    }
}

}

using namespace mrbf;

extern "C" {

const char *mrbf_version(void) { return "mrbf 0.1.0 (gfx950)"; }

const char *mrbf_last_error(const mrbf_ctx *ctx) { return ctx ? ctx->err.c_str() : g_init_err.c_str(); }

int32_t mrbf_init(int32_t device_id, mrbf_ctx **out) {
    if (!out) return -2;
    *out = nullptr;
    int ndev = 0;
    hipError_t e = hipGetDeviceCount(&ndev);
    if (e != hipSuccess || ndev <= 0) {
        (void)hipGetLastError();
        return fail(nullptr, MRBF_ENODEVICE, "no HIP device visible (%s); libmrbf has no CPU path",
                    e == hipSuccess ? "device count 0" : hipGetErrorString(e));
    }
    if (device_id < 0) {
        if (hipGetDevice(&device_id) != hipSuccess) device_id = 0;
    }
    if (device_id >= ndev) return fail(nullptr, -1, "device_id %d out of range (%d devices)", device_id, ndev);
    mrbf_ctx *ctx = new mrbf_ctx();
    ctx->device = device_id;
    auto bail = [&](int code, const char *what) {
        std::string msg = std::string(what) + " failed";
        delete ctx;
        return fail(nullptr, code, "%s", msg.c_str());
    };
    if (hipSetDevice(device_id) != hipSuccess) return bail(MRBF_EHIP, "hipSetDevice");
    if (hipStreamCreateWithFlags(&ctx->own_stream, hipStreamNonBlocking) != hipSuccess)
        return bail(MRBF_EHIP, "hipStreamCreate");
    ctx->stream = ctx->own_stream;
    if (hipHostMalloc(reinterpret_cast<void **>(&ctx->hpin), 64 * sizeof(unsigned long long), hipHostMallocDefault) != hipSuccess) {
        (void)hipGetLastError();
        ctx->hpin = nullptr;
    }
    if (hipHostMalloc(reinterpret_cast<void **>(&ctx->pin_base), PIN_BYTES, hipHostMallocDefault) != hipSuccess) {
        (void)hipGetLastError();
        ctx->pin_base = nullptr;
    }
    if (rocblas_create_handle(&ctx->blas) != rocblas_status_success) return bail(MRBF_EBLAS, "rocblas_create_handle");
    rocblas_set_stream(ctx->blas, ctx->stream);
    rocblas_set_pointer_mode(ctx->blas, rocblas_pointer_mode_host);
    for (auto &ev : ctx->ev)
        if (hipEventCreate(&ev) != hipSuccess) return bail(MRBF_EHIP, "hipEventCreate");
    {
        int lo = 0, hi = 0;
        (void)hipDeviceGetStreamPriorityRange(&lo, &hi);
        if (hipStreamCreateWithPriority(&ctx->panel_stream, hipStreamNonBlocking, hi) != hipSuccess)
            return bail(MRBF_EHIP, "hipStreamCreateWithPriority");
    }
    for (auto &ev : ctx->evx)
        if (hipEventCreateWithFlags(&ev, hipEventDisableTiming) != hipSuccess) return bail(MRBF_EHIP, "hipEventCreate");
    {
        if (const char *bg = mrbf_env("MRBF_BULK_GRID")) ctx->bulk_grid = atoi(bg);
        if (const char *e = mrbf_env("MRBF_CHOL_IMPL")) ctx->chol_impl = atoi(e);
        ctx->mega = mega_knobs_from_env();
        if (const char *e = mrbf_env("MRBF_SPIN_MS")) ctx->spin_ms = std::max(1, atoi(e));
        hipDeviceProp_t prop;
        int ncu = 256;
        bool gfx950 = false;
        if (hipGetDeviceProperties(&prop, device_id) == hipSuccess) {
            ncu = prop.multiProcessorCount;
            gfx950 = std::strncmp(prop.gcnArchName, "gfx950", 6) == 0;
        }
        ctx->ncu = ncu;
        ctx->small_cluster_ok = (gfx950 && ncu == 256) ? 1 : 0;
        const char *env = mrbf_env("MRBF_BULK_RESERVE");
        const int reserve_per_32 = env ? atoi(env) : 0;
        std::vector<uint32_t> mask((ncu + 31) / 32, 0u);
        for (int cu = 0; cu < ncu; ++cu)
            if ((cu % 32) < 32 - reserve_per_32) mask[cu / 32] |= (1u << (cu % 32));
        if (reserve_per_32 > 0 && hipExtStreamCreateWithCUMask(&ctx->bulk_stream, (uint32_t)mask.size(), mask.data()) == hipSuccess) {
            ctx->bulk_masked = 1;
        } else {
            (void)hipGetLastError();
            if (hipStreamCreateWithFlags(&ctx->bulk_stream, hipStreamNonBlocking) != hipSuccess) return bail(MRBF_EHIP, "hipStreamCreate");
        }
    }
    *out = ctx;
    return MRBF_OK;
}

int32_t mrbf_shutdown(mrbf_ctx *ctx) {
    if (!ctx) return -1;
    (void)hipSetDevice(ctx->device);
    (void)hipStreamSynchronize(ctx->stream);
    for (auto &b : ctx->slots)
        if (b.p) (void)hipFree(b.p);
    for (auto &b : ctx->model_pool)
        if (b.p) (void)hipFree(b.p);
    for (auto &t : ctx->mega_tables)
        if (t.block) (void)hipFree(t.block);
    if (ctx->hpin) (void)hipHostFree(ctx->hpin);
    if (ctx->pin_base) (void)hipHostFree(ctx->pin_base);
    for (auto &ev : ctx->ev)
        if (ev) (void)hipEventDestroy(ev);
    for (auto &ev : ctx->evx)
        if (ev) (void)hipEventDestroy(ev);
    if (ctx->panel_stream) {
        (void)hipStreamSynchronize(ctx->panel_stream);
        (void)hipStreamDestroy(ctx->panel_stream);
    }
    if (ctx->bulk_stream) {
        (void)hipStreamSynchronize(ctx->bulk_stream);
        (void)hipStreamDestroy(ctx->bulk_stream);
    }
    if (ctx->blas) rocblas_destroy_handle(ctx->blas);
    if (ctx->own_stream) (void)hipStreamDestroy(ctx->own_stream);
    delete ctx;
    return MRBF_OK;
}

int32_t mrbf_set_option(mrbf_ctx *ctx, int32_t key, double value) {
    if (!ctx) return -1;
    int v = (int)value;
    switch (key) {
        case MRBF_OPT_GRAM_MODE: ctx->gram_mode = v; break;
        case MRBF_OPT_RESIDUAL: ctx->residual = v; break;
        case MRBF_OPT_FORCE_PATH: ctx->force_path = v; break;
        case MRBF_OPT_CHOL_IMPL: ctx->chol_impl = v; break;
        case MRBF_OPT_EVAL_IMPL: ctx->eval_impl = v; break;
        case MRBF_OPT_TIMING: ctx->timing = v; break;
        case MRBF_OPT_DIAG_IMPL: ctx->diag_impl = v; break;
        case MRBF_OPT_CHOL_WINDOW: ctx->chol_window = v; break;
        case MRBF_OPT_SPIN_MS: ctx->spin_ms = v > 0 ? v : 1000; break;
        case MRBF_OPT_DEBUG_FAULT: ctx->debug_fault = v; break;
        case MRBF_OPT_SMALL_FIT_MAX_N:
            if (!(value >= 512.0 && value <= 2048.0)) return fail(ctx, -2, "MRBF_OPT_SMALL_FIT_MAX_N: %g is not in 512 .. 2048", value);
            ctx->small_fit_max_n = v;
            break;
        case MRBF_OPT_SMALL_LU:
            if (!(value == 0.0 || value == 1.0)) return fail(ctx, -2, "MRBF_OPT_SMALL_LU: %g is not 0 or 1", value);
            ctx->small_lu = v;
            break;
        default: return fail(ctx, -2, "unknown option key %d", key);
    }
    return MRBF_OK;
}

int32_t mrbf_get_option(const mrbf_ctx *ctx, int32_t key, double *value) {
    if (!ctx) return -1;
    if (!value) return -3;
    switch (key) {
        case MRBF_OPT_GRAM_MODE: *value = ctx->gram_mode; break;
        case MRBF_OPT_RESIDUAL: *value = ctx->residual; break;
        case MRBF_OPT_FORCE_PATH: *value = ctx->force_path; break;
        case MRBF_OPT_CHOL_IMPL: *value = ctx->chol_impl; break;
        case MRBF_OPT_EVAL_IMPL: *value = ctx->eval_impl; break;
        case MRBF_OPT_TIMING: *value = ctx->timing; break;
        case MRBF_OPT_DIAG_IMPL: *value = ctx->diag_impl; break;
        case MRBF_OPT_CHOL_WINDOW: *value = ctx->chol_window; break;
        case MRBF_OPT_SPIN_MS: *value = ctx->spin_ms; break;
        case MRBF_OPT_DEBUG_FAULT: *value = ctx->debug_fault; break;
        case MRBF_OPT_SMALL_FIT_MAX_N: *value = ctx->small_fit_max_n; break;
        case MRBF_OPT_SMALL_LU: *value = ctx->small_lu; break;
        case MRBF_OPT_LAST_DEVICE_MS: *value = ctx->last_device_ms; break;
        case MRBF_OPT_SLOW_LAUNCHES: *value = ctx->slow_launches; break;
        case MRBF_OPT_ARENA_BYTES: {
            double bytes = 0.0;
            for (int i = 0; i < S_NSLOTS; ++i) bytes += (double)ctx->slots[i].bytes;
            for (auto &b : ctx->model_pool) bytes += (double)b.bytes;
            *value = bytes;
            break;
        }
        case MRBF_OPT_LIVE_HANDLES: *value = ctx->live_models + ctx->live_round4 + ctx->live_dbs; break;
        default: return -2;
    }
    return MRBF_OK;
}

int32_t mrbf_set_stream(mrbf_ctx *ctx, void *hip_stream) {
    if (!ctx) return -1;
    (void)hipSetDevice(ctx->device);
    MRBF_HIP(ctx, hipStreamSynchronize(ctx->stream));
    ctx->stream = hip_stream ? (hipStream_t)hip_stream : ctx->own_stream;
    MRBF_BLAS(ctx, rocblas_set_stream(ctx->blas, ctx->stream));
    return MRBF_OK;
}

int32_t mrbf_sync(mrbf_ctx *ctx) {
    if (!ctx) return -1;
    MRBF_HIP(ctx, hipStreamSynchronize(ctx->stream));
    return MRBF_OK;
}

}
```

morbit.jl_amd/csrc/gram_fused.hip:

```cpp
#include "radial.hpp"

namespace mrbf {

typedef double v4d __attribute__((ext_vector_type(4)));
typedef double v2d __attribute__((ext_vector_type(2)));

constexpr int GW_LDT = 66;

template <int KID, bool FAST>
__global__ __launch_bounds__(256, 2) void gram_w_kernel(const double *__restrict__ Xc, const double *__restrict__ sq, int64_t n,
                                                        int64_t npad, double *__restrict__ Phi, int64_t ld, KP p, int nt, int nseg,
                                                        int seglen, double *__restrict__ Wpart, double *__restrict__ rspart, int dbg) {
    __shared__ __attribute__((aligned(16))) double T[2][64 * GW_LDT];
    __shared__ double Tsq[2][64];
    const int tid = threadIdx.x, lane = tid & 63, wave = tid >> 6;
    const int l15 = lane & 15, l4 = lane >> 4;
    const int seg = blockIdx.x % nseg, I = nt - 1 - (int)(blockIdx.x / nseg);
    const int jt0 = seg * seglen;
    const int jt1 = (jt0 + seglen < nt) ? jt0 + seglen : nt;
    const int64_t iw0 = (int64_t)I * 128 + 32 * wave;
    double bI[2][16];
#pragma unroll
    for (int it = 0; it < 2; ++it)
#pragma unroll
        for (int ks = 0; ks < 16; ++ks) bI[it][ks] = Xc[(iw0 + it * 16 + l15) * 64 + ks * 4 + l4];
    double sqi[2];
#pragma unroll
    for (int it = 0; it < 2; ++it) sqi[it] = sq[iw0 + it * 16 + l15];
    v4d wacc[4][2];
#pragma unroll
    for (int tt = 0; tt < 4; ++tt)
#pragma unroll
        for (int it = 0; it < 2; ++it) wacc[tt][it] = (v4d){0.0, 0.0, 0.0, 0.0};
    double rs[2] = {0.0, 0.0};
    const int nh = 2 * (jt1 - jt0);
    if (nh > 0) {
        const double *src = Xc + (int64_t)jt0 * 128 * 64;
        const double *ssq = sq + (int64_t)jt0 * 128;
        v2d pf[4];
        double pfsq = 0.0;
        if (tid < 64) pfsq = ssq[tid];
#pragma unroll 1
        for (int half = 0; half < 2; ++half) {
#pragma unroll
            for (int u = 0; u < 4; ++u) pf[u] = *(const v2d *)(src + (tid + 256 * (4 * half + u)) * 2);
#pragma unroll
            for (int u = 0; u < 4; ++u) {
                const int e = (tid + 256 * (4 * half + u)) * 2;
                *(v2d *)&T[0][(e >> 6) * GW_LDT + (e & 63)] = pf[u];
            }
        }
        if (tid < 64) Tsq[0][tid] = pfsq;
        __syncthreads();
#pragma unroll 1
        for (int h = 0; h < nh; ++h) {
            const int buf = h & 1;
            const double *Tb = T[buf];
            const int64_t jb = (int64_t)jt0 * 128 + 64 * h;
            const bool store = (jt0 + (h >> 1)) <= I && !(dbg & 1);
            const bool full = jb + 64 <= n && (int64_t)I * 128 + 128 <= n;
            const bool edge = jb + 64 > n || (jt0 + (h >> 1)) == I;
            const bool more = h + 1 < nh && !(dbg & 16);
            const double *s2 = src + (int64_t)(h + 1) * 64 * 64;
            if (more && tid < 64) pfsq = ssq[64 * (h + 1) + tid];
#pragma unroll 1
            for (int sub = 0; sub < 2; ++sub) {
                const double *Ts = Tb + sub * 32 * GW_LDT;
                if (more) {
#pragma unroll
                    for (int u = 0; u < 4; ++u) pf[u] = *(const v2d *)(s2 + (tid + 256 * (4 * sub + u)) * 2);
                }
                v4d acc[2][2];
#pragma unroll
                for (int jt = 0; jt < 2; ++jt)
#pragma unroll
                    for (int it = 0; it < 2; ++it) acc[jt][it] = (v4d){0.0, 0.0, 0.0, 0.0};
                if (!(dbg & 8))
#pragma unroll
                for (int ks = 0; ks < 16; ++ks) {
                    double a[2];
#pragma unroll
                    for (int jt = 0; jt < 2; ++jt) a[jt] = Ts[(jt * 16 + l15) * GW_LDT + ks * 4 + l4];
#pragma unroll
                    for (int jt = 0; jt < 2; ++jt)
#pragma unroll
                        for (int it = 0; it < 2; ++it)
                            acc[jt][it] = __builtin_amdgcn_mfma_f64_16x16x4f64(a[jt], bI[it][ks], acc[jt][it], 0, 0, 0);
                }
                if (more) {
#pragma unroll
                    for (int u = 0; u < 4; ++u) {
                        const int e = (tid + 256 * (4 * sub + u)) * 2;
                        *(v2d *)&T[buf ^ 1][(e >> 6) * GW_LDT + (e & 63)] = pf[u];
                    }
                    if (sub == 0 && tid < 64) Tsq[buf ^ 1][tid] = pfsq;
                }
                if (edge || !FAST) {
#pragma unroll
                    for (int jt = 0; jt < 2; ++jt)
#pragma unroll
                        for (int r = 0; r < 4; ++r) {
                            const int jl = sub * 32 + jt * 16 + l4 + 4 * r;
                            const int64_t gj = jb + jl;
                            const double sqj = Tsq[buf][jl];
#pragma unroll
                            for (int it = 0; it < 2; ++it) {
                                const int64_t gi = iw0 + it * 16 + l15;
                                double s = fma(-2.0, acc[jt][it][r], sqi[it] + sqj);
                                s = s > 0.0 ? s : 0.0;
                                if (gi == gj) s = 0.0;
                                double v = (dbg & 2) ? s : rbf_phi_t<KID, FAST>(s, p);
                                v = gj < n ? v : 0.0;
                                acc[jt][it][r] = v;
                                rs[it] += v;
                            }
                        }
                } else {
#pragma unroll
                    for (int jt = 0; jt < 2; ++jt)
#pragma unroll
                        for (int r = 0; r < 4; ++r) {
                            const double sqj = Tsq[buf][sub * 32 + jt * 16 + l4 + 4 * r];
#pragma unroll
                            for (int it = 0; it < 2; ++it) {
                                double s = fma(-2.0, acc[jt][it][r], sqi[it] + sqj);
                                s = s > 0.0 ? s : 0.0;
                                const double v = (dbg & 2) ? s : rbf_phi_t<KID, FAST>(s, p);
                                acc[jt][it][r] = v;
                                rs[it] += v;
                            }
                        }
                }
                if (store) {
                    double *dst = Phi + (jb + sub * 32 + l4) * ld + iw0 + l15;
                    if (full) {
#pragma unroll
                        for (int jt = 0; jt < 2; ++jt)
#pragma unroll
                            for (int r = 0; r < 4; ++r)
#pragma unroll
                                for (int it = 0; it < 2; ++it) dst[(int64_t)(jt * 16 + 4 * r) * ld + it * 16] = acc[jt][it][r];
                    } else {
#pragma unroll
                        for (int jt = 0; jt < 2; ++jt)
#pragma unroll
                            for (int r = 0; r < 4; ++r)
#pragma unroll
                                for (int it = 0; it < 2; ++it) {
                                    const int64_t gj = jb + sub * 32 + jt * 16 + l4 + 4 * r, gi = iw0 + it * 16 + l15;
                                    if (gi < n && gj < n) dst[(int64_t)(jt * 16 + 4 * r) * ld + it * 16] = acc[jt][it][r];
                                }
                    }
                }
                if (!(dbg & 4))
#pragma unroll
                for (int jt = 0; jt < 2; ++jt) {
#pragma unroll
                    for (int r = 0; r < 4; ++r) {
                        double aw[4];
#pragma unroll
                        for (int tt = 0; tt < 4; ++tt) aw[tt] = Ts[(jt * 16 + 4 * r + l4) * GW_LDT + tt * 16 + l15];
#pragma unroll
                        for (int tt = 0; tt < 4; ++tt)
#pragma unroll
                            for (int it = 0; it < 2; ++it)
                                wacc[tt][it] = __builtin_amdgcn_mfma_f64_16x16x4f64(aw[tt], acc[jt][it][r], wacc[tt][it], 0, 0, 0);
                    }
                }
            }
            __syncthreads();
        }
    }
#pragma unroll
    for (int tt = 0; tt < 4; ++tt)
#pragma unroll
        for (int r = 0; r < 4; ++r) {
            const int t = tt * 16 + l4 + 4 * r;
#pragma unroll
            for (int it = 0; it < 2; ++it) Wpart[((int64_t)seg * 64 + t) * npad + iw0 + it * 16 + l15] = wacc[tt][it][r];
        }
#pragma unroll
    for (int it = 0; it < 2; ++it) {
        double x = rs[it];
        x += __shfl_xor(x, 16);
        x += __shfl_xor(x, 32);
        if (l4 == 0) rspart[(int64_t)seg * npad + iw0 + it * 16 + l15] = x;
    }
}

__device__ __forceinline__ double sum_partials(const double *__restrict__ p, int cnt, int64_t stride) {
    double sp[8] = {0.0, 0.0, 0.0, 0.0, 0.0, 0.0, 0.0, 0.0};
    int c = 0;
    for (; c + 32 <= cnt; c += 32) {
        double v[32];
#pragma unroll
        for (int u = 0; u < 32; ++u) v[u] = p[(int64_t)(c + u) * stride];
#pragma unroll
        for (int u = 0; u < 32; ++u) sp[u & 7] += v[u];
    }
    for (; c + 8 <= cnt; c += 8) {
        double v[8];
#pragma unroll
        for (int u = 0; u < 8; ++u) v[u] = p[(int64_t)(c + u) * stride];
#pragma unroll
        for (int u = 0; u < 8; ++u) sp[u] += v[u];
    }
    for (int u = 0; c + u < cnt; ++u) sp[u] += p[(int64_t)(c + u) * stride];
    return ((sp[0] + sp[1]) + (sp[2] + sp[3])) + ((sp[4] + sp[5]) + (sp[6] + sp[7]));
}

constexpr int PJ_LS = 68;
constexpr int PJ_QP = 80;

__device__ __forceinline__ v4d pj_tile(const double *As, const double *Bs, int mt, int nt, int K, int l15, int l4) {
    v4d acc = {0.0, 0.0, 0.0, 0.0};
    const double *ap = As + (mt * 16 + l15) * PJ_LS + l4;
    const double *bp = Bs + (nt * 16 + l15) * PJ_LS + l4;
    for (int k = 0; k < K; k += 4) acc = __builtin_amdgcn_mfma_f64_16x16x4f64(ap[k], bp[k], acc, 0, 0, 0);
    return acc;
}

__global__ __launch_bounds__(256) void proj_reduce_kernel(const double *__restrict__ Wpart, const double *__restrict__ rspart, int nseg,
                                                          int64_t npad, int64_t n, int d, int q, const double *__restrict__ linv,
                                                          const double *__restrict__ Q1, double rsqrtn, double *__restrict__ W1,
                                                          double *__restrict__ Gp, double *__restrict__ trp) {
    __shared__ double Ws[64 * PJ_LS];
    __shared__ double Ls[64 * PJ_LS];
    __shared__ double W1s[PJ_QP * PJ_LS];
    __shared__ double Qs[PJ_QP * PJ_LS];
    const int tid = threadIdx.x, i = tid & 63, g = tid >> 6;
    const int lane = tid & 63, wave = tid >> 6, l15 = lane & 15, l4 = lane >> 4;
    const int64_t R0 = (int64_t)blockIdx.x * 64;
    const bool live = R0 + i < n;
    constexpr int Q4 = PJ_QP / 4;
    double qv[Q4];
#pragma unroll
    for (int u = 0; u < Q4; ++u) {
        const int a = g + 4 * u;
        qv[u] = (a < q && live) ? Q1[R0 + i + (int64_t)a * npad] : 0.0;
    }
    const double rsv = (g == 0 && live) ? sum_partials(rspart + R0 + i, nseg, npad) * rsqrtn : 0.0;
    if (q > 1) {
        double lv[16];
#pragma unroll
        for (int u = 0; u < 16; ++u) {
            const int e = tid + 256 * u, c = e & 63, t = e >> 6;
            lv[u] = (c < d && t <= c) ? linv[c + (int64_t)t * 128] : 0.0;
        }
#pragma unroll
        for (int half = 0; half < 2; ++half) {
            double sv[8] = {0.0, 0.0, 0.0, 0.0, 0.0, 0.0, 0.0, 0.0};
            for (int s0 = 0; s0 < nseg; s0 += 8) {
                double wv[8][8];
#pragma unroll
                for (int u = 0; u < 8; ++u)
#pragma unroll
                    for (int sgm = 0; sgm < 8; ++sgm) {
                        const int t = g * 16 + half * 8 + u;
                        wv[u][sgm] = s0 + sgm < nseg ? Wpart[((int64_t)(s0 + sgm) * 64 + t) * npad + R0 + i] : 0.0;
                    }
#pragma unroll
                for (int u = 0; u < 8; ++u)
                    sv[u] += ((wv[u][0] + wv[u][1]) + (wv[u][2] + wv[u][3])) + ((wv[u][4] + wv[u][5]) + (wv[u][6] + wv[u][7]));
            }
#pragma unroll
            for (int u = 0; u < 8; ++u) Ws[i * PJ_LS + (g * 16 + half * 8 + u)] = live ? sv[u] : 0.0;
        }
#pragma unroll
        for (int u = 0; u < 16; ++u) {
            const int e = tid + 256 * u;
            Ls[(e & 63) * PJ_LS + (e >> 6)] = lv[u];
        }
    }
#pragma unroll
    for (int u = 0; u < Q4; ++u) {
        const int a = g + 4 * u;
        Qs[a * PJ_LS + i] = qv[u];
        if (a > d || q == 1) W1s[a * PJ_LS + i] = 0.0;
    }
    if (g == 0) {
        W1s[i] = rsv;
        W1[R0 + i] = rsv;
    }
    __syncthreads();
    if (q > 1) {
#pragma unroll 1
        for (int tile = wave; tile < 16; tile += 4) {
            const int ct = tile >> 2, it = tile & 3;
            const v4d acc = pj_tile(Ls, Ws, ct, it, 64, l15, l4);
#pragma unroll
            for (int r = 0; r < 4; ++r) {
                const int c = ct * 16 + l4 + 4 * r, ii = it * 16 + l15;
                if (c < d) {
                    W1s[(1 + c) * PJ_LS + ii] = acc[r];
                    W1[R0 + ii + (int64_t)(1 + c) * npad] = acc[r];
                }
            }
        }
    }
    __syncthreads();
    double *out = Gp + (size_t)blockIdx.x * q * q;
    const int qt = (q + 15) >> 4;
#pragma unroll 1
    for (int tile = wave; tile < qt * qt; tile += 4) {
        const int at = tile % qt, bt = tile / qt;
        const v4d acc = pj_tile(Qs, W1s, at, bt, 64, l15, l4);
#pragma unroll
        for (int r = 0; r < 4; ++r) {
            const int a = at * 16 + l4 + 4 * r, bb = bt * 16 + l15;
            if (a < q && bb < q) out[a + bb * q] = acc[r];
            if (at == bt && a == bb && a < q) Ls[a] = acc[r];
        }
    }
    __syncthreads();
    if (tid == 0) {
        double tr = 0.0;
        for (int a = 0; a < q; ++a) tr += Ls[a];
        trp[blockIdx.x] = tr;
    }
}

__global__ __launch_bounds__(256) void proj_shift_kernel(const double *__restrict__ Gp, const double *__restrict__ trp, int nchunks, int q,
                                                         double nphi0, double nmq, double *__restrict__ G, double *__restrict__ Mh,
                                                         double *__restrict__ scal, int *__restrict__ flags) {
    __shared__ double dg[256];
    __shared__ double smu;
    const int tid = threadIdx.x;
    const size_t qq = (size_t)q * q;
    const int idx = blockIdx.x * 256 + tid;
    const double *p0 = Gp + (idx < (int)qq ? idx : 0);
    double tv = 0.0;
    for (int c = tid; c < nchunks; c += 256) tv += trp[c];
    double s0[8] = {0, 0, 0, 0, 0, 0, 0, 0};
    int c = 0;
    for (; c + 64 <= nchunks; c += 64) {
        double v0[64];
#pragma unroll
        for (int u = 0; u < 64; ++u) v0[u] = p0[(size_t)(c + u) * qq];
#pragma unroll
        for (int u = 0; u < 64; ++u) s0[u & 7] += v0[u];
    }
    for (; c < nchunks; ++c) s0[c & 7] += p0[(size_t)c * qq];
    const double gv = ((s0[0] + s0[1]) + (s0[2] + s0[3])) + ((s0[4] + s0[5]) + (s0[6] + s0[7]));
    dg[tid] = tv;
    __syncthreads();
    for (int w = 128; w > 0; w >>= 1) {
        if (tid < w) dg[tid] += dg[tid + w];
        __syncthreads();
    }
    if (tid == 0) {
        const double tr = dg[0];
        const double mu = (nphi0 - tr) / nmq;
        const bool ok = mu > 0.0 && mu < 1e300;
        smu = ok ? mu : 1.0;
        if (blockIdx.x == 0) {
            scal[0] = tr;
            scal[1] = smu;
            flags[2] = ok ? 0 : 1;
        }
    }
    __syncthreads();
    if (idx < (int)qq) {
        G[idx] = gv;
        Mh[idx] = 0.5 * gv + ((idx % q) == (idx / q) ? 0.5 * smu : 0.0);
    }
}

__global__ __launch_bounds__(256) void proj_panels_kernel(const double *__restrict__ Q1, const double *__restrict__ W1,
                                                          const double *__restrict__ Mh, int64_t n, int64_t npad, int q, int K2, int skip,
                                                          double *__restrict__ PA, double *__restrict__ PB, double *__restrict__ v0) {
    __shared__ double Qs[64 * PJ_LS];
    __shared__ double Ms[PJ_QP * PJ_LS];
    const int tid = threadIdx.x, i = tid & 63, g = tid >> 6;
    const int lane = tid & 63, wave = tid >> 6, l15 = lane & 15, l4 = lane >> 4;
    const int64_t R0 = (int64_t)blockIdx.x * 64;
    const bool live = R0 + i < n;
    constexpr int QA = 17;
    double qv[QA];
#pragma unroll
    for (int u = 0; u < QA; ++u) {
        const int a = g + 4 * u;
        qv[u] = (a < q && live) ? Q1[R0 + i + (int64_t)a * npad] : 0.0;
    }
    constexpr int ME = (PJ_QP * PJ_LS + 255) / 256;
    double mv[ME];
#pragma unroll
    for (int u = 0; u < ME; ++u) {
        const int e = tid + 256 * u, bb = e / PJ_LS, a = e % PJ_LS;
        mv[u] = (a < q && bb < q) ? Mh[a + bb * q] : 0.0;
    }
#pragma unroll
    for (int u = 0; u < ME; ++u) {
        const int e = tid + 256 * u;
        if (e < PJ_QP * PJ_LS) Ms[e] = mv[u];
    }
#pragma unroll
    for (int u = 0; u < QA; ++u) Qs[i * PJ_LS + g + 4 * u] = qv[u];
    __syncthreads();
    const int qq = q - skip, qt = (q + 15) >> 4, K = (q + 3) & ~3;
#pragma unroll 1
    for (int tile = wave; tile < qt * 4; tile += 4) {
        const int bt = tile >> 2, it = tile & 3;
        const v4d acc = pj_tile(Ms, Qs, bt, it, K, l15, l4);
        const int ii = it * 16 + l15;
        const bool lv = R0 + ii < n;
        double w1[4], qb[4];
#pragma unroll
        for (int r = 0; r < 4; ++r) {
            const int b = bt * 16 + l4 + 4 * r;
            w1[r] = (b < q && lv) ? W1[R0 + ii + (int64_t)b * npad] : 0.0;
            qb[r] = b < q ? Qs[ii * PJ_LS + b] : 0.0;
        }
#pragma unroll
        for (int r = 0; r < 4; ++r) {
            const int b = bt * 16 + l4 + 4 * r;
            if (b >= q) continue;
            const double v = lv ? w1[r] - acc[r] : 0.0;
            if (b >= skip) {
                const int c = b - skip;
                PA[R0 + ii + (int64_t)c * npad] = qb[r];
                PB[R0 + ii + (int64_t)c * npad] = v;
                PA[R0 + ii + (int64_t)(qq + c) * npad] = v;
                PB[R0 + ii + (int64_t)(qq + c) * npad] = qb[r];
            } else {
                v0[R0 + ii] = v;
            }
        }
    }
    for (int c = 2 * qq + g; c < K2; c += 4) {
        PA[R0 + i + (int64_t)c * npad] = 0.0;
        PB[R0 + i + (int64_t)c * npad] = 0.0;
    }
}

bool gram_w_applies(const mrbf_ctx *ctx, const mrbf_model *M) {
    static const int on = mrbf_env("MRBF_GRAM_FUSED") ? atoi(mrbf_env("MRBF_GRAM_FUSED")) : 1;
    if (!on || ctx->gram_mode != 0) return false;
    if (M->dpad != 64 || M->q < 1 || M->q > 65 || M->n < 1024) return false;
    if (kp_nonsmooth(M->kp)) return false;
    return M->kp.fast || M->kp.kid == MRBF_GAUSSIAN || M->kp.kid == MRBF_THIN_PLATE_SPLINE;
}

int launch_gram_w(mrbf_ctx *ctx, const mrbf_model *M, double *Phi, int64_t ld, double **Wpart_out, double **rspart_out, int *nseg_out) {
    const int nt = (int)(M->npad / 128);
    static const int dbg = mrbf_env("MRBF_GW_DBG") ? atoi(mrbf_env("MRBF_GW_DBG")) : 0;
    static const int wgs = mrbf_env("MRBF_GW_WGS") ? atoi(mrbf_env("MRBF_GW_WGS")) : 512;
    int nseg = wgs / nt;
    if (nseg < 1) nseg = 1;
    if (nseg > nt) nseg = nt;
    const int seglen = (nt + nseg - 1) / nseg;
    nseg = (nt + seglen - 1) / seglen;
    double *Wpart, *rspart;
    MRBF_TRY(get_buf(ctx, S_GW_PART, (size_t)nseg * 64 * M->npad, &Wpart));
    MRBF_TRY(get_buf(ctx, S_GW_RS, (size_t)nseg * M->npad, &rspart));
    const dim3 grid((unsigned)(nt * nseg));
    if (M->kp.fast) {
        MRBF_DISPATCH_KID(M->kp.kid, hipLaunchKernelGGL((gram_w_kernel<KID, true>), grid, dim3(256), 0, ctx->stream, M->Xc, M->sq, M->n,
                                                        M->npad, Phi, ld, M->kp, nt, nseg, seglen, Wpart, rspart, dbg));
    } else if (M->kp.kid == MRBF_GAUSSIAN) {
        hipLaunchKernelGGL((gram_w_kernel<MRBF_GAUSSIAN, false>), grid, dim3(256), 0, ctx->stream, M->Xc, M->sq, M->n, M->npad, Phi, ld,
                           M->kp, nt, nseg, seglen, Wpart, rspart, dbg);
    } else {
        hipLaunchKernelGGL((gram_w_kernel<MRBF_THIN_PLATE_SPLINE, false>), grid, dim3(256), 0, ctx->stream, M->Xc, M->sq, M->n, M->npad,
                           Phi, ld, M->kp, nt, nseg, seglen, Wpart, rspart, dbg);
    }
    MRBF_HIP(ctx, hipGetLastError());
    *Wpart_out = Wpart;
    *rspart_out = rspart;
    *nseg_out = nseg;
    return 0;
}

int launch_projection_small(mrbf_ctx *ctx, const mrbf_model *M, const double *Wpart, const double *rspart, int nseg, const double *linv,
                            const double *Q1, double *W1, double *G, double *scal, int *flags, int K2, int skip, double *PA, double *PB,
                            double *v0) {
    const int64_t n = M->n, npad = M->npad;
    const int q = M->q, nch = (int)(npad / 64);
    double *Gp, *Mh;
    MRBF_TRY(get_buf(ctx, S_GW_GP, (size_t)nch * q * q + nch, &Gp));
    MRBF_TRY(get_buf(ctx, S_GW_M, (size_t)q * q, &Mh));
    double *trp = Gp + (size_t)nch * q * q;
    hipLaunchKernelGGL(proj_reduce_kernel, dim3((unsigned)nch), dim3(256), 0, ctx->stream, Wpart, rspart, nseg, npad, n, M->d, q, linv, Q1,
                       1.0 / std::sqrt((double)n), W1, Gp, trp);
    hipLaunchKernelGGL(proj_shift_kernel, dim3((unsigned)((q * q + 255) / 256)), dim3(256), 0, ctx->stream, Gp, trp, nch, q,
                       (double)n * M->kp.phi0, (double)std::max<int64_t>(n - q, 1), G, Mh, scal, flags);
    hipLaunchKernelGGL(proj_panels_kernel, dim3((unsigned)nch), dim3(256), 0, ctx->stream, Q1, W1, Mh, n, npad, q, K2, skip, PA, PB, v0);
    MRBF_HIP(ctx, hipGetLastError());
    return 0;
}

}
```

morbit.jl_amd/csrc/solve.hip:

```cpp
#include "common.hpp"
#include "small.hpp"

namespace mrbf {

__global__ void fit_publish_kernel(const int *__restrict__ dinfo, const double *__restrict__ scal, const unsigned long long *__restrict__ dstat,
                                   int *__restrict__ hflags, double *__restrict__ hscal, unsigned long long *__restrict__ hstat) {
    const int t = threadIdx.x;
    if (t < 4) hflags[t] = dinfo[t];
    if (t >= 4 && t < 6 && scal) hscal[t - 4] = scal[t - 4];
    if (t == 6 && dstat && hstat) hstat[0] = dstat[0];
}

__global__ void fill_saddle_kernel(const double *__restrict__ Pi, int64_t n, int q, double *__restrict__ S, int64_t N) {
    const int64_t idx = (int64_t)blockIdx.x * blockDim.x + threadIdx.x;
    const int64_t tot = n * q;
    if (idx < tot) {
        const int64_t i = idx % n;
        const int t = (int)(idx / n);
        const double v = Pi[idx];
        S[i + (n + t) * N] = v;
        S[(n + t) + i * N] = v;
    } else if (idx < tot + (int64_t)q * q) {
        const int64_t r = idx - tot;
        S[(n + r % q) + (n + r / q) * N] = 0.0;
// ... 504 lines not shown
            for (int u = 0; u < 32; ++u) v[u] = c0 + u < nch ? part[(size_t)(c0 + u) * 2 * k * q + e] : 0.0;
#pragma unroll
            for (int u = 0; u < 32; ++u) sv += v[u];
        }
        if (e < k * q)
            t2[e] = sv;
        else
            zz[e - k * q] = sv;
    }
    __syncthreads();
    for (int e = tid; e < k * q; e += nthr) {
        const int l = e / q, a = e % q;
        double corr = 0.0;
        for (int b0 = 0; b0 < q; b0 += 16) {
            double gv[16];
#pragma unroll
            for (int u = 0; u < 16; ++u) gv[u] = b0 + u < q ? G[b0 + u + (int64_t)a * q] : 0.0;
#pragma unroll
            for (int u = 0; u < 16; ++u) corr = fma(gv[u], b0 + u < q ? t2[l * q + b0 + u] : 0.0, corr);
        }
        zz[e] = T1[a + (int64_t)l * q] - zz[e] + cg * corr;
        T2[a + (int64_t)l * q] = t2[e];
    }
    __syncthreads();
    for (int e = tid; e < k * d; e += nthr) {
        const int l = e / d, j = e % d;
        double acc = 0.0;
        for (int i0 = j; i0 < d; i0 += 16) {
            double iv[16];
#pragma unroll
            for (int u = 0; u < 16; ++u) iv[u] = i0 + u < d ? LxInv[i0 + u + (int64_t)j * 128] : 0.0;
#pragma unroll
            for (int u = 0; u < 16; ++u) acc = fma(iv[u], i0 + u < d ? zz[l * q + 1 + i0 + u] : 0.0, acc);
        }
        xx[l * q + 1 + j] = acc;
    }
    __syncthreads();
    if (tid < k) {
        const int l = tid;
        double dsum = 0.0;
        for (int t0 = 1; t0 < q; t0 += 16) {
            double mv[16];
#pragma unroll
            for (int u = 0; u < 16; ++u) mv[u] = t0 + u < q ? mean[t0 + u - 1] : 0.0;
#pragma unroll
            for (int u = 0; u < 16; ++u) dsum = fma(mv[u], t0 + u < q ? xx[l * q + t0 + u] : 0.0, dsum);
        }
        xx[l * q] = zz[l * q] / sqrtn - dsum;
    }
    __syncthreads();
    for (int e = tid; e < k * q; e += nthr) lam_out[(e % q) + (int64_t)(e / q) * q] = xx[e];
}

__global__ __launch_bounds__(256) void tail_apply_kernel(const double *__restrict__ Bw, int64_t ldb, const double *__restrict__ Q1, int64_t ldq,
                                                         const double *__restrict__ T2, const double *__restrict__ lamsrc, int64_t n,
                                                         int64_t npad, int q, int k, double *__restrict__ W, double *__restrict__ Wc,
                                                         double *__restrict__ lam) {
    __shared__ double part4[4][64];
    const int tid = threadIdx.x, r = tid & 63, g = tid >> 6;
    const int64_t row = (int64_t)blockIdx.x * 64 + r;
    for (int l = 0; l < k; ++l) {
        double s0 = 0.0, s1 = 0.0;
        if (row < n) {
            int t = g;
            for (; t + 4 < q; t += 8) {
                s0 = fma(Q1[row + (int64_t)t * ldq], T2[t + (int64_t)l * q], s0);
                s1 = fma(Q1[row + (int64_t)(t + 4) * ldq], T2[t + 4 + (int64_t)l * q], s1);
            }
            if (t < q) s0 = fma(Q1[row + (int64_t)t * ldq], T2[t + (int64_t)l * q], s0);
        }
        __syncthreads();
        part4[g][r] = s0 + s1;
        __syncthreads();
        if (g == 0 && row < npad) {
            const double v = row < n ? Bw[row + (int64_t)l * ldb] - ((part4[0][r] + part4[1][r]) + (part4[2][r] + part4[3][r])) : 0.0;
            Wc[row + (int64_t)l * npad] = v;
            if (row < n) W[row * k + l] = v;
        }
    }
    if (blockIdx.x == 0)
        for (int e = tid; e < q * k; e += 256) lam[(int64_t)(e % q) * k + e / q] = lamsrc[(e % q) + (int64_t)(e / q) * q];
}

static int fit_chol(mrbf_ctx *ctx, mrbf_model *M, const double *Y, mrbf_fit_info *info, int *not_pd, int *gave_up, int impl = 0) {
    const int64_t n = M->n, npad = M->npad;
    const int k = M->k, q = M->q, d = M->d;
    const double one = 1.0, mhalf = -0.5;
    *not_pd = 0;
    *gave_up = 0;
    if (impl == 0) impl = ctx->chol_impl;
    const bool builtin = impl != 1;
    PotrfOpts popt;
    popt.impl = impl;
    const int xt = builtin ? (int)round_up(k, 128) : 0;
    const int64_t ld = npad + xt;
    double *Phi, *B;
    int *dinfo;
    MRBF_TRY(get_buf(ctx, S_PHI, (size_t)ld * npad, &Phi));
    MRBF_TRY(get_buf(ctx, S_RHS, (size_t)npad * k, &B));
    MRBF_TRY(get_buf(ctx, S_INFO, (size_t)4, &dinfo));
    MRBF_HIP(ctx, hipMemsetAsync(dinfo, 0, 4 * sizeof(int), ctx->stream));
    const bool tailq = q > 1 && tail_basis_applies(M) && M->k == k;
    if (!tailq) hipLaunchKernelGGL(rhs_from_values_kernel, dim3(nblk(npad * k)), dim3(256), 0, ctx->stream, Y, n, k, B, npad);
    double *Q1 = nullptr, *Wm = nullptr, *G = nullptr, *T1 = nullptr, *scal = nullptr, *Tall = nullptr, *LxInv = nullptr;
    int64_t lt = 0, dq = 0;
    info->mu = 0.0;
    hipStream_t main_stream = ctx->stream;
    const bool side = q > 0 && ctx->panel_stream && ctx->panel_stream != main_stream && n >= 2048;
    const bool fused = q > 0 && gram_w_applies(ctx, M) && (q == 1 || round_up(d, 128) == 128);
    if (q > 0) {
        MRBF_TRY(get_buf(ctx, S_Q1, (size_t)npad * q, &Q1));
        MRBF_TRY(get_buf(ctx, S_W1, (size_t)npad * q, &Wm));
        MRBF_TRY(get_buf(ctx, S_G, (size_t)q * q, &G));
        MRBF_TRY(get_buf(ctx, S_T1, (size_t)q * k, &T1));
        MRBF_TRY(get_buf(ctx, S_MISC, (size_t)8, &scal));
        if (side) {
            MRBF_HIP(ctx, hipEventRecord(ctx->evx[0], main_stream));
            MRBF_HIP(ctx, hipStreamWaitEvent(ctx->panel_stream, ctx->evx[0], 0));
            ctx->stream = ctx->panel_stream;
        }
        struct RestoreStream {
            mrbf_ctx *c;
            hipStream_t s;
            ~RestoreStream() { c->stream = s; }
        } restore{ctx, main_stream};
        if (tailq) {
            double *scratch;
            MRBF_TRY(get_buf(ctx, S_PI, tail_basis_scratch_doubles(), &scratch));
            MRBF_TRY(get_buf(ctx, S_QR_INV, (size_t)128 * 128, &LxInv));
            MRBF_TRY(launch_tail_basis(ctx, M, Y, scratch, LxInv, T1, Q1, B, builtin ? Phi : nullptr, ld, xt, dinfo));
        } else if (q > 1) {
            dq = round_up(d, 128);
            lt = dq + npad;
            MRBF_TRY(get_buf(ctx, S_PI, (size_t)lt * dq, &Tall));
            MRBF_HIP(ctx, hipMemsetAsync(Tall, 0, (size_t)lt * dq * sizeof(double), ctx->stream));
            hipLaunchKernelGGL(xc_to_tall_kernel, dim3(nblk(n * d)), dim3(256), 0, ctx->stream, M->Xc, n, d, M->dpad, Tall, lt, dq);
            MRBF_TRY(tsmm_tn(ctx, n, d, d, 1.0, Tall + dq, lt, Tall + dq, lt, 0.0, Tall, lt));
            MRBF_TRY(launch_pad_identity(ctx, Tall, d, dq, lt));
            if (dq == 128) MRBF_TRY(get_buf(ctx, S_QR_INV, (size_t)128 * 128, &LxInv));
            MRBF_TRY(potrf_blocked_tall(ctx, dq, lt, Tall, lt, dinfo + 1, LxInv, popt));
        }
        if (!tailq) hipLaunchKernelGGL(build_q1_kernel, dim3(nblk(npad * q)), dim3(256), 0, ctx->stream, Tall, lt, dq, n, npad, q, Q1);
        if (!fused) MRBF_HIP(ctx, hipMemsetAsync(Wm, 0, (size_t)npad * q * sizeof(double), ctx->stream));
        if (!tailq) {
            MRBF_TRY(tsmm_tn(ctx, n, q, k, 1.0, Q1, npad, B, npad, 0.0, T1, q));
            hipLaunchKernelGGL(sub_qt_kernel, dim3((unsigned)((n + 63) / 64)), dim3(256), 0, ctx->stream, B, npad, Q1, npad, T1, n, q, k);
            if (builtin) hipLaunchKernelGGL(set_rhs_rows_kernel, dim3(nblk(npad * xt)), dim3(256), 0, ctx->stream, Phi, ld, npad, xt, B, k);
        }
        if (side) MRBF_HIP(ctx, hipEventRecord(ctx->evx[1], ctx->stream));
    }
    ctx->stream = main_stream;
    MRBF_HIP(ctx, hipEventRecord(ctx->ev[0], ctx->stream));
    double *Wpart = nullptr, *rspart = nullptr;
    int nseg = 0;
    if (fused)
        MRBF_TRY(launch_gram_w(ctx, M, Phi, ld, &Wpart, &rspart, &nseg));
    else
        MRBF_TRY(launch_gram(ctx, ctx->gram_mode, M->C, M->Xc, M->sq, n, M->npad, M->d, M->dpad, M->kp, Phi, ld));
    MRBF_HIP(ctx, hipEventRecord(ctx->ev[1], ctx->stream));
    if (side) MRBF_HIP(ctx, hipStreamWaitEvent(ctx->stream, ctx->evx[1], 0));
    if (fused) {
        const int skip = (q > 1 && round_up(2 * (q - 1), 16) < round_up(2 * q, 16)) ? 1 : 0;
        const int K2 = (int)round_up(2 * (q - skip), 16);
        double *PA, *PB, *v0 = nullptr;
        MRBF_TRY(get_buf(ctx, S_STAGE_C, (size_t)npad * K2, &PA));
        MRBF_TRY(get_buf(ctx, S_STAGE_D, (size_t)npad * K2, &PB));
        if (skip) MRBF_TRY(get_buf(ctx, S_V0, (size_t)npad, &v0));
        MRBF_TRY(launch_projection_small(ctx, M, Wpart, rspart, nseg, LxInv, Q1, Wm, G, scal, dinfo, K2, skip, PA, PB, v0));
        MRBF_TRY(launch_update_lower(ctx, PA, npad, PB, npad, Phi, ld, npad / 128, K2, v0, 1.0 / std::sqrt((double)n), n));
    } else if (q > 0) {
        MRBF_TRY(symm_panel(ctx, n, npad, q, Phi, ld, Q1, npad, Wm, npad, true, 1.0 / std::sqrt((double)n)));
        MRBF_TRY(tsmm_tn(ctx, n, q, q, 1.0, Q1, npad, Wm, npad, 0.0, G, q));
        hipLaunchKernelGGL(trace_kernel, dim3(1), dim3(256), 0, ctx->stream, G, q, scal);
        MRBF_BLAS(ctx, rocblas_dgemm(ctx->blas, rocblas_operation_none, rocblas_operation_none, (int)n, q, q, &mhalf, Q1, (int)npad,
                                     G, q, &one, Wm, (int)npad));
        hipLaunchKernelGGL(shift_from_trace_kernel, dim3(1), dim3(1), 0, ctx->stream, scal, (double)n * M->kp.phi0,
                           (double)std::max<int64_t>(n - q, 1), dinfo);
        const int skip = (q > 1 && round_up(2 * (q - 1), 16) < round_up(2 * q, 16)) ? 1 : 0;
        const int K2 = (int)round_up(2 * (q - skip), 16);
        double *PA, *PB, *v0 = nullptr;
        MRBF_TRY(get_buf(ctx, S_STAGE_C, (size_t)npad * K2, &PA));
        MRBF_TRY(get_buf(ctx, S_STAGE_D, (size_t)npad * K2, &PB));
        if (skip) MRBF_TRY(get_buf(ctx, S_V0, (size_t)npad, &v0));
        hipLaunchKernelGGL(build_panels_kernel, dim3(nblk(npad * K2)), dim3(256), 0, ctx->stream, Q1, Wm, scal, n, npad, q, K2, skip, PA, PB, v0);
        MRBF_TRY(launch_update_lower(ctx, PA, npad, PB, npad, Phi, ld, npad / 128, K2, v0, 1.0 / std::sqrt((double)n), n));
    }
    MRBF_HIP(ctx, hipEventRecord(ctx->ev[2], ctx->stream));
    int hinfo = 0;
    double *linv_all = nullptr;
    if (builtin) {
        MRBF_TRY(get_buf(ctx, S_CHOL_WS, (size_t)npad * 128, &linv_all));
        MRBF_TRY(launch_pad_identity(ctx, Phi, n, npad, ld));
        if (q == 0) hipLaunchKernelGGL(set_rhs_rows_kernel, dim3(nblk(npad * xt)), dim3(256), 0, ctx->stream, Phi, ld, npad, xt, B, k);
        popt.xreal = k;
        popt.info_clean = true;
        MRBF_TRY(potrf_blocked_tall(ctx, npad, npad + xt, Phi, ld, dinfo, linv_all, popt));
        MRBF_HIP(ctx, hipEventRecord(ctx->ev[3], ctx->stream));
    } else {
        int *dpot;
        MRBF_TRY(get_buf(ctx, S_IPIV, (size_t)4, &dpot));
        MRBF_BLAS(ctx, rocsolver_dpotrf(ctx->blas, rocblas_fill_lower, (int)n, Phi, (int)ld, dpot));
        MRBF_HIP(ctx, hipMemcpyAsync(dinfo, dpot, sizeof(int), hipMemcpyDeviceToDevice, ctx->stream));
        MRBF_HIP(ctx, hipEventRecord(ctx->ev[3], ctx->stream));
    }
    double *T1w = nullptr;
    if (q > 0) MRBF_TRY(get_buf(ctx, S_T1W, (size_t)q * k, &T1w));
    auto solve_tail = [&](bool persistent) -> int {
        if (builtin) {
            hipLaunchKernelGGL(get_rhs_rows_kernel, dim3(nblk(npad * k)), dim3(256), 0, ctx->stream, Phi, ld, npad, B, k);
            if (persistent)
                MRBF_TRY(backsolve_persistent(ctx, npad, Phi, ld, linv_all, B, npad, k, dinfo + 3));
            else
                MRBF_TRY(backsolve_blocked(ctx, npad, Phi, ld, linv_all, B, npad, k));
        } else {
            MRBF_BLAS(ctx, rocsolver_dpotrs(ctx->blas, rocblas_fill_lower, (int)n, k, Phi, (int)ld, B, (int)npad));
        }
        static const int tail3 = mrbf_env("MRBF_TAIL3") ? atoi(mrbf_env("MRBF_TAIL3")) : 1;
        if (tail3 && q > 0 && q <= 129 && k <= 16 && (q == 1 || LxInv)) {
            const int nch = (int)(npad / 64);
            double *T2, *part;
            MRBF_TRY(get_buf(ctx, S_T2, (size_t)q * k, &T2));
            MRBF_TRY(get_buf(ctx, S_TAIL_PART, (size_t)nch * 2 * k * q, &part));
            hipLaunchKernelGGL(tail_dots_kernel, dim3((unsigned)nch), dim3(256), 0, ctx->stream, B, npad, Q1, Wm, npad, n, q, k, part);
            hipLaunchKernelGGL(tail_coeff_kernel, dim3(1), dim3(1024), 0, ctx->stream, part, nch, q, k, q > 1 ? d : 0, T1, G, fused ? 1.0 : 0.5, LxInv,
                               std::sqrt((double)n), M->mean, T2, T1w);
            hipLaunchKernelGGL(tail_apply_kernel, dim3((unsigned)nch), dim3(256), 0, ctx->stream, B, npad, Q1, npad, T2, T1w, n, M->npad, q, k, M->W,
                               M->Wc, M->lam);
            MRBF_HIP(ctx, hipGetLastError());
            return 0;
        }
        if (q > 0) {
            double *T2;
            MRBF_TRY(get_buf(ctx, S_T2, (size_t)q * k, &T2));
            MRBF_HIP(ctx, hipMemcpyAsync(T1w, T1, (size_t)q * k * sizeof(double), hipMemcpyDeviceToDevice, ctx->stream));
            MRBF_TRY(tsmm_tn(ctx, n, q, k, 1.0, Q1, npad, B, npad, 0.0, T2, q));
            hipLaunchKernelGGL(sub_qt_kernel, dim3((unsigned)((n + 63) / 64)), dim3(256), 0, ctx->stream, B, npad, Q1, npad, T2, n, q, k);
            MRBF_TRY(tsmm_tn(ctx, n, q, k, -1.0, Wm, npad, B, npad, 1.0, T1w, q));
            if (q > 1) {
                if (LxInv)
                    hipLaunchKernelGGL(apply_linv_t_kernel, dim3(1), dim3(256), 0, ctx->stream, LxInv, d, T1w + 1, (int64_t)q, k);
                else if (d <= 256)
                    hipLaunchKernelGGL(trsm_lt_small_kernel, dim3(1), dim3(256), 0, ctx->stream, Tall, lt, d, T1w + 1, (int64_t)q, k);
                else
                    MRBF_BLAS(ctx, rocblas_dtrsm(ctx->blas, rocblas_side_left, rocblas_fill_lower, rocblas_operation_transpose,
                                                 rocblas_diagonal_non_unit, d, k, &one, Tall, (int)lt, T1w + 1, q));
            }
            hipLaunchKernelGGL(finish_lambda_kernel, dim3((unsigned)k), dim3(64), 0, ctx->stream, T1w, q, k, std::sqrt((double)n), M->mean);
        }
        hipLaunchKernelGGL(scatter_solution_kernel, dim3(nblk(M->npad * k + (int64_t)q * k)), dim3(256), 0, ctx->stream, B, npad, n,
                           M->npad, k, q, (int64_t)0, M->W, M->Wc, M->lam, T1w ? T1w : B, (int64_t)q);
        MRBF_HIP(ctx, hipGetLastError());
        return 0;
    };
    MRBF_TRY(solve_tail(true));
    MRBF_HIP(ctx, hipEventRecord(ctx->ev[4], ctx->stream));
    {
        int hflags_local[4] = {0, 0, 0, 0};
        double hscal_local[2] = {0.0, 0.0};
        int *hflags = ctx->hpin ? reinterpret_cast<int *>(ctx->hpin + HPIN_FIT_FLAGS) : hflags_local;
        double *hscal = ctx->hpin ? reinterpret_cast<double *>(ctx->hpin + HPIN_FIT_SCAL) : hscal_local;
        hscal[0] = hscal[1] = 0.0;
        static const int publish = mrbf_env("MRBF_FIT_PUBLISH") ? atoi(mrbf_env("MRBF_FIT_PUBLISH")) : 1;
        if (ctx->hpin && publish) {
            unsigned long long *hstat = nullptr;
            const unsigned long long *dstat = nullptr;
            if (ctx->mega_stat_pending && ctx->mega_stat_dev) {
                ctx->hpin[HPIN_MEGA_STAT] = ~0ull;
                hstat = &ctx->hpin[HPIN_MEGA_STAT];
                dstat = ctx->mega_stat_dev;
                ctx->mega_stat_pending = 2;
            }
            hipLaunchKernelGGL(fit_publish_kernel, dim3(1), dim3(64), 0, ctx->stream, (const int *)dinfo, q > 0 ? (const double *)scal : nullptr, dstat,
                               hflags, hscal, hstat);
        } else {
        MRBF_HIP(ctx, hipMemcpyAsync(hflags, dinfo, 4 * sizeof(int), hipMemcpyDeviceToHost, ctx->stream));
        if (q > 0) MRBF_HIP(ctx, hipMemcpyAsync(hscal, scal, 2 * sizeof(double), hipMemcpyDeviceToHost, ctx->stream));
        MRBF_TRY(mega_stat_enqueue(ctx));
        }
        MRBF_HIP(ctx, hipStreamSynchronize(ctx->stream));
        MRBF_TRY(mega_stat_finish(ctx));
        info->ms_factor_device = ctx->last_device_ms;
        hinfo = hflags[0];
        if (hinfo < 0) {
            *gave_up = 1;
            info->giveup_code = -hinfo;
            return 0;
        }
        info->factor_info = hinfo;
        if (q > 0) info->mu = hscal[1];
        if (hflags[1] < 0) {
            *gave_up = 1;
            info->giveup_code = -hflags[1];
            return 0;
        }
        if (hflags[1] != 0) {
            *not_pd = 1;
            info->factor_info = -2;
            return 0;
        }
        if (hflags[2] != 0) {
            *not_pd = 1;
            info->factor_info = -1;
            return 0;
        }
        if (hinfo != 0) {
            *not_pd = 1;
            return 0;
        }
        if (hflags[3] != 0) {
            info->fallbacks |= MRBF_FB_BACKSOLVE_BLOCKED;
            info->giveup_code = hflags[3];
            MRBF_TRY(solve_tail(false));
            MRBF_HIP(ctx, hipEventRecord(ctx->ev[4], ctx->stream));
        }
    }
    MRBF_HIP(ctx, hipEventSynchronize(ctx->ev[4]));
    MRBF_HIP(ctx, hipEventElapsedTime(&info->ms_gram, ctx->ev[0], ctx->ev[1]));
    MRBF_HIP(ctx, hipEventElapsedTime(&info->ms_project, ctx->ev[1], ctx->ev[2]));
    MRBF_HIP(ctx, hipEventElapsedTime(&info->ms_factor, ctx->ev[2], ctx->ev[3]));
    MRBF_HIP(ctx, hipEventElapsedTime(&info->ms_solve, ctx->ev[3], ctx->ev[4]));
    info->path = q > 0 ? MRBF_PATH_PROJ_CHOL : MRBF_PATH_CHOL;
// ... 224 lines not shown
```

Baseline: 175.6.

## Balance fused Gram work with a piece partition and split the update tail

Replaces the fixed segment-per-strip grid of the fused Gram+W kernel with a host-planned, cached partition. Each workgroup walks a list of (strip, first tile, count, slot) pieces sized to about two workgroups per CU. A separate mirror kernel handles the upper-triangle contributions, and the partials are indexed by slot through a device table. The lower-triangular Cholesky update also now splits a small remainder wave of tiles into 32x32 subtile blocks, so the last partial wave is spread across more workgroups. The cost is an extra kernel launch, a one-time table upload per shape, and more complicated indexing.

```diff
diff --git a/include/mrbf.h b/include/mrbf.h
--- a/include/mrbf.h
+++ b/include/mrbf.h
@@ -327,6 +327,10 @@
 int32_t mrbf_debug_mega_tables2(int32_t nt, int32_t mt, int32_t slack, int32_t slack_chain, int32_t first, int32_t win, int32_t srows,
                                 int32_t half_cols, const int32_t *opt5, int64_t *out6);
 int32_t mrbf_debug_mega_plan(int32_t nt, int32_t mt, int32_t xreal, int64_t *out39);
+int32_t mrbf_debug_gram_partition(int32_t nt, int32_t wgs, int32_t *counts5, int32_t *pieces, int64_t cap_pieces, int32_t *wgrow,
+                                  int64_t cap_wgrow, int32_t *sidx);
+int32_t mrbf_debug_update_lower(mrbf_ctx *ctx, int32_t nt, int32_t K2, double *C_inout, const double *PA, const double *PB,
+                                const double *v0, double cs, int64_t cn, int32_t form);
 
 enum { MRBF_PS_OK = 0, MRBF_PS_CRITICAL = 1, MRBF_PS_FAILURE = 2 };
 typedef struct {
diff --git a/morbit.jl_amd/_lib.py b/morbit.jl_amd/_lib.py
--- a/morbit.jl_amd/_lib.py
+++ b/morbit.jl_amd/_lib.py
@@ -302,6 +302,9 @@
     "mrbf_debug_mega_tables": (ctypes.c_int32, [ctypes.c_int32] * 8 + [c_vp]),
     "mrbf_debug_mega_tables2": (ctypes.c_int32, [ctypes.c_int32] * 8 + [c_vp, c_vp]),
     "mrbf_debug_mega_plan": (ctypes.c_int32, [ctypes.c_int32] * 3 + [c_vp]),
+    "mrbf_debug_gram_partition": (ctypes.c_int32, [ctypes.c_int32, ctypes.c_int32, c_vp, c_vp, ctypes.c_int64, c_vp, ctypes.c_int64, c_vp]),
+    "mrbf_debug_update_lower": (ctypes.c_int32, [c_vp, ctypes.c_int32, ctypes.c_int32, c_vp, c_vp, c_vp, c_vp, ctypes.c_double,
+                                                 ctypes.c_int64, ctypes.c_int32]),
     "mrbf_stochastic_rank": (ctypes.c_int32, [ctypes.c_int32, c_vp, c_vp, c_vp, ctypes.c_double, c_vp]),
     "mrbf_ps_step": (ctypes.c_int32, [c_vp, c_vp, c_vp, c_vp, c_vp, c_vp, c_vp, ctypes.POINTER(PsOptions), c_vp, c_vp, c_vp,
                                       ctypes.POINTER(PsInfo)]),
diff --git a/morbit.jl_amd/csrc/chol.hip b/morbit.jl_amd/csrc/chol.hip
--- a/morbit.jl_amd/csrc/chol.hip
+++ b/morbit.jl_amd/csrc/chol.hip
@@ -6,6 +6,8 @@
 
 int debug_diag(mrbf_ctx *ctx, const double *A128_dev, int reps, float *ms_per_call, unsigned long long *stamps_host);
 int launch_pad_identity(mrbf_ctx *ctx, double *A, int64_t n, int64_t npad, int64_t ld);
+int launch_update_lower_form(mrbf_ctx *ctx, const double *A, int64_t lda, const double *B, int64_t ldb, double *C, int64_t ldc,
+                             int64_t nt, int K, const double *cvec, double cs, int64_t cn, int form);
 
 int potrf_lower(mrbf_ctx *ctx, int impl, int64_t n, double *A, int64_t lda, int *info_host) {
     int *dinfo;
@@ -84,3 +86,20 @@
                 st[4], st[5]);
     return MRBF_OK;
 }
+
+extern "C" int32_t mrbf_debug_update_lower(mrbf_ctx *ctx, int32_t nt, int32_t K2, double *C, const double *PA, const double *PB,
+                                           const double *v0, double cs, int64_t cn, int32_t form) {
+    if (!ctx) return -1;
+    if (nt <= 0 || nt > 512) return -2;
+    if (K2 <= 0 || (K2 & 15)) return -3;
+    if (!C || !is_device_ptr(C)) return -4;
+    if (!PA || !is_device_ptr(PA)) return -5;
+    if (!PB || !is_device_ptr(PB)) return -6;
+    if (v0 && !is_device_ptr(v0)) return -7;
+    if (form < 0 || form > 2) return -10;
+    (void)hipSetDevice(ctx->device);
+    const int64_t npad = (int64_t)nt * 128;
+    MRBF_TRY(launch_update_lower_form(ctx, PA, npad, PB, npad, C, npad, nt, K2, v0, cs, cn, form));
+    MRBF_HIP(ctx, hipStreamSynchronize(ctx->stream));
+    return MRBF_OK;
+}
diff --git a/morbit.jl_amd/csrc/chol_blocked.hip b/morbit.jl_amd/csrc/chol_blocked.hip
--- a/morbit.jl_amd/csrc/chol_blocked.hip
+++ b/morbit.jl_amd/csrc/chol_blocked.hip
@@ -10,6 +10,66 @@
 
 enum { UPD_LOWER_SUB = 0, UPD_OVERWRITE = 1, UPD_FULL_SUB = 2, UPD_COLUMN_SUB = 3 };
 int launch_diag(mrbf_ctx *ctx, hipStream_t st, double *Ajj, int64_t lda, double *Linv, int *dinfo, int col0);
+
+__device__ __forceinline__ void tri_tile(int bid, int &ti, int &tj) {
+    int t = (int)((sqrt(8.0 * (double)bid + 1.0) - 1.0) * 0.5);
+    while ((t + 1) * (t + 2) / 2 <= bid) ++t;
+    while (t * (t + 1) / 2 > bid) --t;
+    ti = t;
+    tj = bid - t * (t + 1) / 2;
+}
+
+__device__ __forceinline__ void update_subtile(const double *__restrict__ A, int64_t lda, const double *__restrict__ B, int64_t ldb,
+                                               double *__restrict__ C, int64_t ldc, int K, int bid, int sub,
+                                               const double *__restrict__ cvec, double cs, int64_t cn) {
+    const int lane = threadIdx.x & 63, wave = __builtin_amdgcn_readfirstlane(threadIdx.x >> 6);
+    const int l15 = lane & 15, l4 = lane >> 4;
+    int ti, tj;
+    tri_tile(bid, ti, tj);
+    const int si = sub & 3, sj = sub >> 2;
+    if (ti == tj && sj > si) return;
+    const int64_t i0 = (int64_t)ti * 128 + si * 32 + (wave >> 1) * 16, j0 = (int64_t)tj * 128 + sj * 32 + (wave & 1) * 16;
+    const int64_t gi = i0 + l15;
+    v4d acc;
+#pragma unroll
+    for (int r = 0; r < 4; ++r) acc[r] = -C[gi + (j0 + l4 + 4 * r) * ldc];
+    const double *ab = A + i0, *bb = B + j0;
+    const uint32_t aoff = (uint32_t)(l15 + l4 * lda), boff = (uint32_t)(l15 + l4 * ldb);
+#pragma unroll 1
+    for (int k0 = 0; k0 < K; k0 += 128) {
+        double av[32], bv[32];
+#pragma unroll
+        for (int u = 0; u < 32; ++u) {
+            const int k = k0 + 4 * u;
+            av[u] = k < K ? (ab + (int64_t)k * lda)[aoff] : 0.0;
+            bv[u] = k < K ? (bb + (int64_t)k * ldb)[boff] : 0.0;
+        }
+#pragma unroll
+        for (int u = 0; u < 32; ++u)
+            if (k0 + 4 * u < K) acc = __builtin_amdgcn_mfma_f64_16x16x4f64(bv[u], av[u], acc, 0, 0, 0);
+    }
+    double cvi = 0.0, cei = 0.0;
+    if (cvec) {
+        cvi = cs * cvec[gi];
+        cei = gi < cn ? cs : 0.0;
+    }
+#pragma unroll
+    for (int r = 0; r < 4; ++r) {
+        const int64_t gj = j0 + l4 + 4 * r;
+        double x = -acc[r];
+        if (cvec) {
+            const double cvj = cvec[gj], cej = gj < cn ? 1.0 : 0.0;
+            x -= fma(cei, cvj, cvi * cej);
+        }
+        if (ti != tj || gi >= gj) C[gi + gj * ldc] = x;
+    }
+}
+
+__global__ __launch_bounds__(256, 2) void chol_update_subtile_kernel(const double *__restrict__ A, int64_t lda, const double *__restrict__ B,
+                                                                  int64_t ldb, double *__restrict__ C, int64_t ldc, int K, int nfull,
+                                                                  const double *__restrict__ cvec, double cs, int64_t cn) {
+    update_subtile(A, lda, B, ldb, C, ldc, K, nfull + (int)(blockIdx.x >> 4), (int)(blockIdx.x & 15), cvec, cs, cn);
+}
 
 template <int TM, int MODE>
 __global__ __launch_bounds__(256, 2) void chol_update_kernel(const double *__restrict__ A, int64_t lda,
@@ -29,11 +89,7 @@
     if (MODE == UPD_LOWER_SUB) {
         const int ntri = mt_sq * (mt_sq + 1) / 2;
         if (bid < ntri || mt_sq == 0) {
-            int t = (int)((sqrt(8.0 * (double)bid + 1.0) - 1.0) * 0.5);
-            while ((t + 1) * (t + 2) / 2 <= bid) ++t;
-            while (t * (t + 1) / 2 > bid) --t;
-            ti = t;
-            tj = bid - t * (t + 1) / 2;
+            tri_tile(bid, ti, tj);
         } else {
             ti = mt_sq + (bid - ntri) / mt_sq;
             tj = (bid - ntri) % mt_sq;
@@ -388,13 +444,31 @@
     return 0;
 }
 
+int launch_update_lower_form(mrbf_ctx *ctx, const double *A, int64_t lda, const double *B, int64_t ldb, double *C, int64_t ldc,
+                             int64_t nt, int K, const double *cvec, double cs, int64_t cn, int form) {
+    if (nt <= 0 || K <= 0) return 0;
+    const int64_t ntiles = nt * (nt + 1) / 2, slots = 2 * (int64_t)ctx->ncu;
+    const int64_t rem = ntiles % slots;
+    if (form == 2) {
+        hipLaunchKernelGGL(chol_update_subtile_kernel, dim3((unsigned)(16 * ntiles)), dim3(256), 0, ctx->stream, A, lda, B, ldb, C, ldc, K,
+                           0, cvec, cs, cn);
+    } else if (form == 0 && rem > 0 && 2 * rem < slots && ntiles > slots) {
+        const int64_t nfull = ntiles - rem;
+        hipLaunchKernelGGL((chol_update_kernel<128, UPD_LOWER_SUB>), dim3((unsigned)nfull), dim3(256), 0, ctx->stream, A, lda, B, ldb,
+                           C, ldc, K, (const int *)nullptr, (int)nt, 0, cvec, cs, cn);
+        hipLaunchKernelGGL(chol_update_subtile_kernel, dim3((unsigned)(16 * rem)), dim3(256), 0, ctx->stream, A, lda, B, ldb, C, ldc, K,
+                           (int)nfull, cvec, cs, cn);
+    } else {
+        hipLaunchKernelGGL((chol_update_kernel<128, UPD_LOWER_SUB>), dim3((unsigned)ntiles), dim3(256), 0, ctx->stream, A, lda, B, ldb,
+                           C, ldc, K, (const int *)nullptr, (int)nt, 0, cvec, cs, cn);
+    }
+    MRBF_HIP(ctx, hipGetLastError());
+    return 0;
+}
+
 int launch_update_lower(mrbf_ctx *ctx, const double *A, int64_t lda, const double *B, int64_t ldb, double *C, int64_t ldc, int64_t nt,
                         int K, const double *cvec, double cs, int64_t cn) {
-    if (nt <= 0 || K <= 0) return 0;
-    hipLaunchKernelGGL((chol_update_kernel<128, UPD_LOWER_SUB>), dim3((unsigned)(nt * (nt + 1) / 2)), dim3(256), 0, ctx->stream, A,
-                       lda, B, ldb, C, ldc, K, (const int *)nullptr, (int)nt, 0, cvec, cs, cn);
-    MRBF_HIP(ctx, hipGetLastError());
-    return 0;
+    return launch_update_lower_form(ctx, A, lda, B, ldb, C, ldc, nt, K, cvec, cs, cn, 0);
 }
 
 int potrf_blocked_tall(mrbf_ctx *ctx, int64_t ncols, int64_t mrows, double *A, int64_t lda, int *dinfo, double *linv_all, PotrfOpts opt) {
diff --git a/morbit.jl_amd/csrc/common.hpp b/morbit.jl_amd/csrc/common.hpp
--- a/morbit.jl_amd/csrc/common.hpp
+++ b/morbit.jl_amd/csrc/common.hpp
@@ -73,6 +73,16 @@
     void *block, *jobs, *wq;
     int npanel, nbulk, nchainjobs, nwin;
     unsigned long long stamp;
+};
+struct GwPlan {
+    std::vector<int> pieces, wgrow[2], sidx;
+    int nwg[2] = {0, 0};
+};
+void gw_plan(int nt, int wgs, GwPlan &P);
+struct GwTables {
+    int nt, wgs, nslots, nwg[2];
+    void *block;
+    const int *wgrow[2], *sidx;
 };
 struct PotrfOpts {
     int impl = 0;
@@ -132,6 +142,7 @@
     std::map<long, float> mega_best_ms;
     std::vector<mrbf::MegaTables> mega_tables;
     unsigned long long mega_table_clock = 0;
+    std::vector<mrbf::GwTables> gw_tables;
 };
 
 struct mrbf_model {
@@ -241,8 +252,9 @@
                 int d, int dpad, const KP &kp, double *Phi, int64_t ld);
 int launch_cross_gram(mrbf_ctx *ctx, const double *X, int64_t m, const double *C, int64_t n, int d, const KP &kp, double *K);
 bool gram_w_applies(const mrbf_ctx *ctx, const mrbf_model *M);
-int launch_gram_w(mrbf_ctx *ctx, const mrbf_model *M, double *Phi, int64_t ld, double **Wpart_out, double **rspart_out, int *nseg_out);
-int launch_projection_small(mrbf_ctx *ctx, const mrbf_model *M, const double *Wpart, const double *rspart, int nseg, const double *linv,
+int launch_gram_w(mrbf_ctx *ctx, const mrbf_model *M, double *Phi, int64_t ld, double **Wpart_out, double **rspart_out,
+                  const int **sidx_out);
+int launch_projection_small(mrbf_ctx *ctx, const mrbf_model *M, const double *Wpart, const double *rspart, const int *sidx, const double *linv,
                             const double *Q1, double *W1, double *G, double *scal, int *flags, int K2, int skip, double *PA, double *PB,
                             double *v0);
 int eval_model(mrbf_ctx *ctx, const mrbf_model *M, int64_t m, const double *Xdev, double *vals_dev, double *jac_dev,
diff --git a/morbit.jl_amd/csrc/context.hip b/morbit.jl_amd/csrc/context.hip
--- a/morbit.jl_amd/csrc/context.hip
+++ b/morbit.jl_amd/csrc/context.hip
@@ -349,6 +349,8 @@
         if (b.p) (void)hipFree(b.p);
     for (auto &t : ctx->mega_tables)
         if (t.block) (void)hipFree(t.block);
+    for (auto &t : ctx->gw_tables)
+        if (t.block) (void)hipFree(t.block);
     if (ctx->hpin) (void)hipHostFree(ctx->hpin);
     if (ctx->pin_base) (void)hipHostFree(ctx->pin_base);
     for (auto &ev : ctx->ev)
diff --git a/morbit.jl_amd/csrc/gram_fused.hip b/morbit.jl_amd/csrc/gram_fused.hip
--- a/morbit.jl_amd/csrc/gram_fused.hip
+++ b/morbit.jl_amd/csrc/gram_fused.hip
@@ -7,17 +7,24 @@
 
 constexpr int GW_LDT = 66;
 
+struct GwPiece {
+    int strip, first, count, slot;
+};
+
 template <int KID, bool FAST>
 __global__ __launch_bounds__(256, 2) void gram_w_kernel(const double *__restrict__ Xc, const double *__restrict__ sq, int64_t n,
-                                                        int64_t npad, double *__restrict__ Phi, int64_t ld, KP p, int nt, int nseg,
-                                                        int seglen, double *__restrict__ Wpart, double *__restrict__ rspart, int dbg) {
+                                                        double *__restrict__ Phi, int64_t ld, KP p, const GwPiece *__restrict__ pieces,
+                                                        const int *__restrict__ wgrow, double *__restrict__ Wpart,
+                                                        double *__restrict__ rspart, int dbg) {
     __shared__ __attribute__((aligned(16))) double T[2][64 * GW_LDT];
     __shared__ double Tsq[2][64];
     const int tid = threadIdx.x, lane = tid & 63, wave = tid >> 6;
     const int l15 = lane & 15, l4 = lane >> 4;
-    const int seg = blockIdx.x % nseg, I = nt - 1 - (int)(blockIdx.x / nseg);
-    const int jt0 = seg * seglen;
-    const int jt1 = (jt0 + seglen < nt) ? jt0 + seglen : nt;
+    const int row0 = wgrow[blockIdx.x], row1 = wgrow[blockIdx.x + 1];
+#pragma unroll 1
+    for (int row = row0; row < row1; ++row) {
+    const GwPiece pc = pieces[row];
+    const int I = pc.strip, jt0 = pc.first, jt1 = pc.first + pc.count, slot = pc.slot;
     const int64_t iw0 = (int64_t)I * 128 + 32 * wave;
     double bI[2][16];
 #pragma unroll
@@ -57,7 +64,7 @@
             const int buf = h & 1;
             const double *Tb = T[buf];
             const int64_t jb = (int64_t)jt0 * 128 + 64 * h;
-            const bool store = (jt0 + (h >> 1)) <= I && !(dbg & 1);
+            const bool store = !(dbg & 1);
             const bool full = jb + 64 <= n && (int64_t)I * 128 + 128 <= n;
             const bool edge = jb + 64 > n || (jt0 + (h >> 1)) == I;
             const bool more = h + 1 < nh && !(dbg & 16);
@@ -177,36 +184,135 @@
         for (int r = 0; r < 4; ++r) {
             const int t = tt * 16 + l4 + 4 * r;
 #pragma unroll
-            for (int it = 0; it < 2; ++it) Wpart[((int64_t)seg * 64 + t) * npad + iw0 + it * 16 + l15] = wacc[tt][it][r];
+            for (int it = 0; it < 2; ++it) Wpart[((int64_t)slot * 64 + t) * 128 + 32 * wave + it * 16 + l15] = wacc[tt][it][r];
         }
 #pragma unroll
     for (int it = 0; it < 2; ++it) {
         double x = rs[it];
         x += __shfl_xor(x, 16);
         x += __shfl_xor(x, 32);
-        if (l4 == 0) rspart[(int64_t)seg * npad + iw0 + it * 16 + l15] = x;
-    }
-}
-
-__device__ __forceinline__ double sum_partials(const double *__restrict__ p, int cnt, int64_t stride) {
-    double sp[8] = {0.0, 0.0, 0.0, 0.0, 0.0, 0.0, 0.0, 0.0};
-    int c = 0;
-    for (; c + 32 <= cnt; c += 32) {
-        double v[32];
-#pragma unroll
-        for (int u = 0; u < 32; ++u) v[u] = p[(int64_t)(c + u) * stride];
-#pragma unroll
-        for (int u = 0; u < 32; ++u) sp[u & 7] += v[u];
-    }
-    for (; c + 8 <= cnt; c += 8) {
-        double v[8];
-#pragma unroll
-        for (int u = 0; u < 8; ++u) v[u] = p[(int64_t)(c + u) * stride];
-#pragma unroll
-        for (int u = 0; u < 8; ++u) sp[u] += v[u];
-    }
-    for (int u = 0; c + u < cnt; ++u) sp[u] += p[(int64_t)(c + u) * stride];
-    return ((sp[0] + sp[1]) + (sp[2] + sp[3])) + ((sp[4] + sp[5]) + (sp[6] + sp[7]));
+        if (l4 == 0) rspart[(int64_t)slot * 128 + 32 * wave + it * 16 + l15] = x;
+    }
+    }
+}
+
+typedef double v4da __attribute__((ext_vector_type(4), aligned(32)));
+__global__ __launch_bounds__(256, 2) void gram_w_mirror_kernel(const double *__restrict__ Xc, int64_t n, const double *__restrict__ Phi,
+                                                               int64_t ld, const GwPiece *__restrict__ pieces,
+                                                               const int *__restrict__ wgrow, double *__restrict__ Wpart,
+                                                               double *__restrict__ rspart) {
+    __shared__ __attribute__((aligned(16))) double T[2][64 * GW_LDT];
+    const int tid = threadIdx.x, lane = tid & 63, wave = tid >> 6;
+    const int l15 = lane & 15, l4 = lane >> 4;
+    const int row0 = wgrow[blockIdx.x], row1 = wgrow[blockIdx.x + 1];
+#pragma unroll 1
+    for (int row = row0; row < row1; ++row) {
+        const GwPiece pc = pieces[row];
+        const int I = pc.strip, jt0 = pc.first, slot = pc.slot;
+        const int64_t iw0 = (int64_t)I * 128 + 32 * wave;
+        v4d wacc[4][2];
+#pragma unroll
+        for (int tt = 0; tt < 4; ++tt)
+#pragma unroll
+            for (int it = 0; it < 2; ++it) wacc[tt][it] = (v4d){0.0, 0.0, 0.0, 0.0};
+        double rs[2] = {0.0, 0.0};
+        const int nh = 2 * pc.count;
+        const double *src = Xc + (int64_t)jt0 * 128 * 64;
+        const double *pcol = Phi + (int64_t)jt0 * 128 + 4 * l4 + (iw0 + l15) * ld;
+        v4d nb[2][2];
+#pragma unroll
+        for (int it = 0; it < 2; ++it)
+#pragma unroll
+            for (int u = 0; u < 2; ++u) nb[it][u] = *(const v4da *)(pcol + 16 * u + (int64_t)it * 16 * ld);
+        v2d pf[4];
+#pragma unroll 1
+        for (int half = 0; half < 2; ++half) {
+#pragma unroll
+            for (int u = 0; u < 4; ++u) pf[u] = *(const v2d *)(src + (tid + 256 * (4 * half + u)) * 2);
+#pragma unroll
+            for (int u = 0; u < 4; ++u) {
+                const int e = (tid + 256 * (4 * half + u)) * 2;
+                *(v2d *)&T[0][(e >> 6) * GW_LDT + (e & 63)] = pf[u];
+            }
+        }
+        __syncthreads();
+#pragma unroll 1
+        for (int h = 0; h < nh; ++h) {
+            const int buf = h & 1;
+            const int64_t jb = (int64_t)jt0 * 128 + 64 * h;
+            const bool more = h + 1 < nh;
+            const double *s2 = src + (int64_t)(h + 1) * 64 * 64;
+#pragma unroll 1
+            for (int sub = 0; sub < 2; ++sub) {
+                const double *Ts = T[buf] + sub * 32 * GW_LDT;
+                v4d cb[2][2];
+#pragma unroll
+                for (int it = 0; it < 2; ++it)
+#pragma unroll
+                    for (int u = 0; u < 2; ++u) cb[it][u] = nb[it][u];
+                if (more || sub == 0) {
+                    const double *pn = pcol + 64 * h + 32 * (sub + 1);
+#pragma unroll
+                    for (int it = 0; it < 2; ++it)
+#pragma unroll
+                        for (int u = 0; u < 2; ++u) nb[it][u] = *(const v4da *)(pn + 16 * u + (int64_t)it * 16 * ld);
+                }
+                if (more) {
+#pragma unroll
+                    for (int u = 0; u < 4; ++u) pf[u] = *(const v2d *)(s2 + (tid + 256 * (4 * sub + u)) * 2);
+                }
+                if (jb + sub * 32 + 32 > n) {
+#pragma unroll
+                    for (int it = 0; it < 2; ++it)
+#pragma unroll
+                        for (int u = 0; u < 2; ++u)
+#pragma unroll
+                            for (int e = 0; e < 4; ++e)
+                                if (jb + sub * 32 + 16 * u + 4 * l4 + e >= n) cb[it][u][e] = 0.0;
+                }
+#pragma unroll
+                for (int it = 0; it < 2; ++it)
+#pragma unroll
+                    for (int u = 0; u < 2; ++u) rs[it] += (cb[it][u][0] + cb[it][u][1]) + (cb[it][u][2] + cb[it][u][3]);
+#pragma unroll
+                for (int u = 0; u < 2; ++u)
+#pragma unroll
+                    for (int e = 0; e < 4; ++e) {
+                        double aw[4];
+#pragma unroll
+                        for (int tt = 0; tt < 4; ++tt) aw[tt] = Ts[(16 * u + 4 * l4 + e) * GW_LDT + tt * 16 + l15];
+#pragma unroll
+                        for (int tt = 0; tt < 4; ++tt)
+#pragma unroll
+                            for (int it = 0; it < 2; ++it)
+                                wacc[tt][it] = __builtin_amdgcn_mfma_f64_16x16x4f64(aw[tt], cb[it][u][e], wacc[tt][it], 0, 0, 0);
+                    }
+                if (more) {
+#pragma unroll
+                    for (int u = 0; u < 4; ++u) {
+                        const int e = (tid + 256 * (4 * sub + u)) * 2;
+                        *(v2d *)&T[buf ^ 1][(e >> 6) * GW_LDT + (e & 63)] = pf[u];
+                    }
+                }
+            }
+            __syncthreads();
+        }
+#pragma unroll
+        for (int tt = 0; tt < 4; ++tt)
+#pragma unroll
+            for (int r = 0; r < 4; ++r) {
+                const int t = tt * 16 + l4 + 4 * r;
+#pragma unroll
+                for (int it = 0; it < 2; ++it) Wpart[((int64_t)slot * 64 + t) * 128 + 32 * wave + it * 16 + l15] = wacc[tt][it][r];
+            }
+#pragma unroll
+        for (int it = 0; it < 2; ++it) {
+            double x = rs[it];
+            x += __shfl_xor(x, 16);
+            x += __shfl_xor(x, 32);
+            if (l4 == 0) rspart[(int64_t)slot * 128 + 32 * wave + it * 16 + l15] = x;
+        }
+    }
 }
 
 constexpr int PJ_LS = 68;
@@ -220,7 +326,8 @@
     return acc;
 }
 
-__global__ __launch_bounds__(256) void proj_reduce_kernel(const double *__restrict__ Wpart, const double *__restrict__ rspart, int nseg,
+__global__ __launch_bounds__(256) void proj_reduce_kernel(const double *__restrict__ Wpart, const double *__restrict__ rspart,
+                                                          const int *__restrict__ sidx,
                                                           int64_t npad, int64_t n, int d, int q, const double *__restrict__ linv,
                                                           const double *__restrict__ Q1, double rsqrtn, double *__restrict__ W1,
                                                           double *__restrict__ Gp, double *__restrict__ trp) {
@@ -239,7 +346,19 @@
         const int a = g + 4 * u;
         qv[u] = (a < q && live) ? Q1[R0 + i + (int64_t)a * npad] : 0.0;
     }
-    const double rsv = (g == 0 && live) ? sum_partials(rspart + R0 + i, nseg, npad) * rsqrtn : 0.0;
+    const int strip = (int)(blockIdx.x >> 1), ioff = (int)(blockIdx.x & 1) * 64 + i;
+    const int f0 = sidx[4 * strip], c0 = sidx[4 * strip + 1], f1 = sidx[4 * strip + 2], nslot = c0 + sidx[4 * strip + 3];
+    auto slot_of = [&](int s) { return s < c0 ? f0 + s : f1 + (s - c0); };
+    double rsv = 0.0;
+    if (g == 0) {
+        for (int s0 = 0; s0 < nslot; s0 += 8) {
+            double v[8];
+#pragma unroll
+            for (int u = 0; u < 8; ++u) v[u] = s0 + u < nslot ? rspart[(int64_t)slot_of(s0 + u) * 128 + ioff] : 0.0;
+            rsv += ((v[0] + v[1]) + (v[2] + v[3])) + ((v[4] + v[5]) + (v[6] + v[7]));
+        }
+        rsv = live ? rsv * rsqrtn : 0.0;
+    }
     if (q > 1) {
         double lv[16];
 #pragma unroll
@@ -250,15 +369,15 @@
 #pragma unroll
         for (int half = 0; half < 2; ++half) {
             double sv[8] = {0.0, 0.0, 0.0, 0.0, 0.0, 0.0, 0.0, 0.0};
-            for (int s0 = 0; s0 < nseg; s0 += 8) {
+            for (int s0 = 0; s0 < nslot; s0 += 8) {
                 double wv[8][8];
 #pragma unroll
-                for (int u = 0; u < 8; ++u)
-#pragma unroll
-                    for (int sgm = 0; sgm < 8; ++sgm) {
-                        const int t = g * 16 + half * 8 + u;
-                        wv[u][sgm] = s0 + sgm < nseg ? Wpart[((int64_t)(s0 + sgm) * 64 + t) * npad + R0 + i] : 0.0;
-                    }
+                for (int sgm = 0; sgm < 8; ++sgm) {
+                    const bool on = s0 + sgm < nslot;
+                    const double *wp = Wpart + ((int64_t)(on ? slot_of(s0 + sgm) : 0) * 64 + g * 16 + half * 8) * 128 + ioff;
+#pragma unroll
+                    for (int u = 0; u < 8; ++u) wv[u][sgm] = on ? wp[u * 128] : 0.0;
+                }
 #pragma unroll
                 for (int u = 0; u < 8; ++u)
                     sv[u] += ((wv[u][0] + wv[u][1]) + (wv[u][2] + wv[u][3])) + ((wv[u][4] + wv[u][5]) + (wv[u][6] + wv[u][7]));
@@ -441,37 +560,107 @@
     return M->kp.fast || M->kp.kid == MRBF_GAUSSIAN || M->kp.kid == MRBF_THIN_PLATE_SPLINE;
 }
 
-int launch_gram_w(mrbf_ctx *ctx, const mrbf_model *M, double *Phi, int64_t ld, double **Wpart_out, double **rspart_out, int *nseg_out) {
+void gw_plan(int nt, int wgs, GwPlan &P) {
+    P = GwPlan{};
+    P.sidx.assign((size_t)4 * nt, 0);
+    for (int pass = 0; pass < 2; ++pass) {
+        const int64_t total = pass == 0 ? (int64_t)nt * (nt + 1) / 2 : (int64_t)nt * (nt - 1) / 2;
+        const int nwg = (int)std::min<int64_t>(std::max(wgs, 1), total);
+        int s = 0, off = 0;
+        P.wgrow[pass].push_back((int)(P.pieces.size() / 4));
+        for (int w = 0; w < nwg; ++w) {
+            int len = (int)((w + 1) * total / nwg - w * total / nwg);
+            while (len > 0) {
+                const int I = pass == 0 ? nt - 1 - s : s, L = pass == 0 ? I + 1 : nt - 1 - I, first = pass == 0 ? 0 : I + 1;
+                const int take = std::min(len, L - off), slot = (int)(P.pieces.size() / 4);
+                const int v[4] = {I, first + off, take, slot};
+                P.pieces.insert(P.pieces.end(), v, v + 4);
+                if (P.sidx[4 * I + 2 * pass + 1]++ == 0) P.sidx[4 * I + 2 * pass] = slot;
+                off += take;
+                len -= take;
+                if (off == L) ++s, off = 0;
+            }
+            P.wgrow[pass].push_back((int)(P.pieces.size() / 4));
+        }
+        P.nwg[pass] = nwg;
+    }
+}
+
+static int gw_tables(mrbf_ctx *ctx, int nt, int wgs, const GwTables **out) {
+    for (auto &t : ctx->gw_tables)
+        if (t.nt == nt && t.wgs == wgs) {
+            *out = &t;
+            return 0;
+        }
+    if (ctx->gw_tables.size() >= 16) {
+        MRBF_HIP(ctx, hipStreamSynchronize(ctx->stream));
+        for (auto &t : ctx->gw_tables) (void)hipFree(t.block);
+        ctx->gw_tables.clear();
+    }
+    GwPlan P;
+    gw_plan(nt, wgs, P);
+    std::vector<int> img(P.pieces);
+    GwTables t{};
+    t.nt = nt;
+    t.wgs = wgs;
+    t.nslots = (int)(P.pieces.size() / 4);
+    t.nwg[0] = P.nwg[0];
+    t.nwg[1] = P.nwg[1];
+    const size_t o0 = img.size();
+    img.insert(img.end(), P.wgrow[0].begin(), P.wgrow[0].end());
+    const size_t o1 = img.size();
+    img.insert(img.end(), P.wgrow[1].begin(), P.wgrow[1].end());
+    const size_t o2 = img.size();
+    img.insert(img.end(), P.sidx.begin(), P.sidx.end());
+    MRBF_HIP(ctx, hipMalloc(&t.block, img.size() * sizeof(int)));
+    if (hipMemcpy(t.block, img.data(), img.size() * sizeof(int), hipMemcpyHostToDevice) != hipSuccess) {
+        (void)hipFree(t.block);
+        return fail(ctx, MRBF_EHIP, "upload of the Gram partition (nt = %d) failed", nt);
+    }
+    t.wgrow[0] = (const int *)t.block + o0;
+    t.wgrow[1] = (const int *)t.block + o1;
+    t.sidx = (const int *)t.block + o2;
+    ctx->gw_tables.push_back(t);
+    *out = &ctx->gw_tables.back();
+    return 0;
+}
+
+int launch_gram_w(mrbf_ctx *ctx, const mrbf_model *M, double *Phi, int64_t ld, double **Wpart_out, double **rspart_out,
+                  const int **sidx_out) {
     const int nt = (int)(M->npad / 128);
     static const int dbg = mrbf_env("MRBF_GW_DBG") ? atoi(mrbf_env("MRBF_GW_DBG")) : 0;
-    static const int wgs = mrbf_env("MRBF_GW_WGS") ? atoi(mrbf_env("MRBF_GW_WGS")) : 512;
-    int nseg = wgs / nt;
-    if (nseg < 1) nseg = 1;
-    if (nseg > nt) nseg = nt;
-    const int seglen = (nt + nseg - 1) / nseg;
-    nseg = (nt + seglen - 1) / seglen;
+    static const int wgs_env = mrbf_env("MRBF_GW_WGS") ? atoi(mrbf_env("MRBF_GW_WGS")) : 0;
+    const int wgs = wgs_env > 0 ? wgs_env : 2 * ctx->ncu;
+    if ((ld & 3) || (reinterpret_cast<uintptr_t>(Phi) & 31))
+        return fail(ctx, MRBF_EHIP, "the fused Gram assembly needs 32-byte aligned columns (ld = %lld)", (long long)ld);
+    const GwTables *t;
+    MRBF_TRY(gw_tables(ctx, nt, wgs, &t));
+    const GwPiece *pieces = (const GwPiece *)t->block;
     double *Wpart, *rspart;
-    MRBF_TRY(get_buf(ctx, S_GW_PART, (size_t)nseg * 64 * M->npad, &Wpart));
-    MRBF_TRY(get_buf(ctx, S_GW_RS, (size_t)nseg * M->npad, &rspart));
-    const dim3 grid((unsigned)(nt * nseg));
+    MRBF_TRY(get_buf(ctx, S_GW_PART, (size_t)t->nslots * 64 * 128, &Wpart));
+    MRBF_TRY(get_buf(ctx, S_GW_RS, (size_t)t->nslots * 128, &rspart));
+    const dim3 grid((unsigned)t->nwg[0]);
     if (M->kp.fast) {
         MRBF_DISPATCH_KID(M->kp.kid, hipLaunchKernelGGL((gram_w_kernel<KID, true>), grid, dim3(256), 0, ctx->stream, M->Xc, M->sq, M->n,
-                                                        M->npad, Phi, ld, M->kp, nt, nseg, seglen, Wpart, rspart, dbg));
+                                                        Phi, ld, M->kp, pieces, t->wgrow[0], Wpart, rspart, dbg));
     } else if (M->kp.kid == MRBF_GAUSSIAN) {
-        hipLaunchKernelGGL((gram_w_kernel<MRBF_GAUSSIAN, false>), grid, dim3(256), 0, ctx->stream, M->Xc, M->sq, M->n, M->npad, Phi, ld,
-                           M->kp, nt, nseg, seglen, Wpart, rspart, dbg);
+        hipLaunchKernelGGL((gram_w_kernel<MRBF_GAUSSIAN, false>), grid, dim3(256), 0, ctx->stream, M->Xc, M->sq, M->n, Phi, ld, M->kp,
+                           pieces, t->wgrow[0], Wpart, rspart, dbg);
     } else {
-        hipLaunchKernelGGL((gram_w_kernel<MRBF_THIN_PLATE_SPLINE, false>), grid, dim3(256), 0, ctx->stream, M->Xc, M->sq, M->n, M->npad,
-                           Phi, ld, M->kp, nt, nseg, seglen, Wpart, rspart, dbg);
-    }
+        hipLaunchKernelGGL((gram_w_kernel<MRBF_THIN_PLATE_SPLINE, false>), grid, dim3(256), 0, ctx->stream, M->Xc, M->sq, M->n, Phi, ld,
+                           M->kp, pieces, t->wgrow[0], Wpart, rspart, dbg);
+    }
+    if (t->nwg[1] > 0)
+        hipLaunchKernelGGL(gram_w_mirror_kernel, dim3((unsigned)t->nwg[1]), dim3(256), 0, ctx->stream, M->Xc, M->n, Phi, ld, pieces,
+                           t->wgrow[1], Wpart, rspart);
     MRBF_HIP(ctx, hipGetLastError());
     *Wpart_out = Wpart;
     *rspart_out = rspart;
-    *nseg_out = nseg;
+    *sidx_out = t->sidx;
     return 0;
 }
 
-int launch_projection_small(mrbf_ctx *ctx, const mrbf_model *M, const double *Wpart, const double *rspart, int nseg, const double *linv,
+int launch_projection_small(mrbf_ctx *ctx, const mrbf_model *M, const double *Wpart, const double *rspart, const int *sidx, const double *linv,
                             const double *Q1, double *W1, double *G, double *scal, int *flags, int K2, int skip, double *PA, double *PB,
                             double *v0) {
     const int64_t n = M->n, npad = M->npad;
@@ -480,7 +669,7 @@
     MRBF_TRY(get_buf(ctx, S_GW_GP, (size_t)nch * q * q + nch, &Gp));
     MRBF_TRY(get_buf(ctx, S_GW_M, (size_t)q * q, &Mh));
     double *trp = Gp + (size_t)nch * q * q;
-    hipLaunchKernelGGL(proj_reduce_kernel, dim3((unsigned)nch), dim3(256), 0, ctx->stream, Wpart, rspart, nseg, npad, n, M->d, q, linv, Q1,
+    hipLaunchKernelGGL(proj_reduce_kernel, dim3((unsigned)nch), dim3(256), 0, ctx->stream, Wpart, rspart, sidx, npad, n, M->d, q, linv, Q1,
                        1.0 / std::sqrt((double)n), W1, Gp, trp);
     hipLaunchKernelGGL(proj_shift_kernel, dim3((unsigned)((q * q + 255) / 256)), dim3(256), 0, ctx->stream, Gp, trp, nch, q,
                        (double)n * M->kp.phi0, (double)std::max<int64_t>(n - q, 1), G, Mh, scal, flags);
@@ -490,3 +679,29 @@
 }
 
 }
+
+extern "C" int32_t mrbf_debug_gram_partition(int32_t nt, int32_t wgs, int32_t *counts5, int32_t *pieces, int64_t cap_pieces, int32_t *wgrow,
+                                             int64_t cap_wgrow, int32_t *sidx) {
+    if (nt < 1 || nt > 4096) return -1;
+    if (wgs < 1) return -2;
+    if (!counts5) return -3;
+    mrbf::GwPlan P;
+    mrbf::gw_plan(nt, wgs, P);
+    const int64_t np = (int64_t)P.pieces.size() / 4, nw = (int64_t)P.wgrow[0].size() + (int64_t)P.wgrow[1].size();
+    counts5[0] = (int32_t)np;
+    counts5[1] = P.nwg[0];
+    counts5[2] = P.nwg[1];
+    counts5[3] = (int32_t)np;
+    counts5[4] = (int32_t)nw;
+    if (pieces) {
+        if (cap_pieces < np) return -5;
+        std::memcpy(pieces, P.pieces.data(), P.pieces.size() * sizeof(int32_t));
+    }
+    if (wgrow) {
+        if (cap_wgrow < nw) return -7;
+        std::memcpy(wgrow, P.wgrow[0].data(), P.wgrow[0].size() * sizeof(int32_t));
+        std::memcpy(wgrow + P.wgrow[0].size(), P.wgrow[1].data(), P.wgrow[1].size() * sizeof(int32_t));
+    }
+    if (sidx) std::memcpy(sidx, P.sidx.data(), P.sidx.size() * sizeof(int32_t));
+    return 0;
+}
diff --git a/morbit.jl_amd/csrc/solve.hip b/morbit.jl_amd/csrc/solve.hip
--- a/morbit.jl_amd/csrc/solve.hip
+++ b/morbit.jl_amd/csrc/solve.hip
@@ -680,9 +680,9 @@
     ctx->stream = main_stream;
     MRBF_HIP(ctx, hipEventRecord(ctx->ev[0], ctx->stream));
     double *Wpart = nullptr, *rspart = nullptr;
-    int nseg = 0;
+    const int *sidx = nullptr;
     if (fused)
-        MRBF_TRY(launch_gram_w(ctx, M, Phi, ld, &Wpart, &rspart, &nseg));
+        MRBF_TRY(launch_gram_w(ctx, M, Phi, ld, &Wpart, &rspart, &sidx));
     else
         MRBF_TRY(launch_gram(ctx, ctx->gram_mode, M->C, M->Xc, M->sq, n, M->npad, M->d, M->dpad, M->kp, Phi, ld));
     MRBF_HIP(ctx, hipEventRecord(ctx->ev[1], ctx->stream));
@@ -694,7 +694,7 @@
         MRBF_TRY(get_buf(ctx, S_STAGE_C, (size_t)npad * K2, &PA));
         MRBF_TRY(get_buf(ctx, S_STAGE_D, (size_t)npad * K2, &PB));
         if (skip) MRBF_TRY(get_buf(ctx, S_V0, (size_t)npad, &v0));
-        MRBF_TRY(launch_projection_small(ctx, M, Wpart, rspart, nseg, LxInv, Q1, Wm, G, scal, dinfo, K2, skip, PA, PB, v0));
+        MRBF_TRY(launch_projection_small(ctx, M, Wpart, rspart, sidx, LxInv, Q1, Wm, G, scal, dinfo, K2, skip, PA, PB, v0));
         MRBF_TRY(launch_update_lower(ctx, PA, npad, PB, npad, Phi, ld, npad / 128, K2, v0, 1.0 / std::sqrt((double)n), n));
     } else if (q > 0) {
         MRBF_TRY(symm_panel(ctx, n, npad, q, Phi, ld, Q1, npad, Wm, npad, true, 1.0 / std::sqrt((double)n)));
```

Result: no change. 176.7, median of 6 (+0.6%).
